# parsakzr/medvae-disentangled-multimodal

Measured on AMD Instinct MI355X. Metric: training images/sec (whole node) + ELBO parity, multimodal CVAE 64×64 bs=256, higher is better.
Workload: dtype fp32 (3xBF16 MFMA, fp32 accumulate); 1 GPU; ConditionalVAE 64x64x3 train step (fwd+loss+bwd+clip+adamw); model=ConditionalVAE, params=927333315, global_batch=256, per_gpu_batch=256, resolution=64, parallelism=dp1, rccl_world_size=1, step_launch=eager

## Files before the change

### include/medvae_hip.h

```cpp
#ifndef MEDVAE_HIP_H
#define MEDVAE_HIP_H

#include <stddef.h>

#ifdef __cplusplus
extern "C" {
#endif

#define MVAE_OK 0
#define MVAE_EINVAL (-1)
#define MVAE_EWORKSPACE (-2)

const char* mvae_last_error(void);
int mvae_abi_version(void);

int mvae_set_math_mode(int mode);
int mvae_get_math_mode(void);
int mvae_set_dropout_salt(const void* salt_dev);

#define MVAE_CONV_WSPLIT 16
#define MVAE_CONV_XSPLIT 32
#define MVAE_CONV_DYSPLIT 64
#define MVAE_CONV_BF16 128
#define MVAE_CONV_PLANAR 256
int mvae_conv2d_nhwc(const float* x, const float* w, const float* bias, const float* residual, float* y,
                     int nb, int h, int w_, int cin, int cout, int kh, int kw, int stride, int pad_t,
                     int pad_l, int ho, int wo, int mode, void* stream);
#define MVAE_CONV_DGRAD_DIRECT 512
int mvae_conv2d_direct32_nhwc(const float* x, const float* w, const float* bias, const float* residual, float* y,
                              int n, int h, int w_, int mode, void* stream);
int mvae_conv2d_ws_nhwc(const float* x, const float* w, const float* bias, const float* residual, float* y,
                        int nb, int h, int w_, int cin, int cout, int kh, int kw, int stride, int pad_t,
                        int pad_l, int ho, int wo, int mode, float* workspace, size_t workspace_bytes, void* stream);
size_t mvae_conv2d_split_workspace_bytes(int nb, int cin, int cout, int kh, int kw, int ho, int wo);
int mvae_conv2d_gnstats_nhwc(const float* x, const float* w, const float* bias, const float* residual, float* y,
                             int nb, int h, int w_, int cin, int cout, int kh, int kw, int stride, int pad_t,
                             int pad_l, int ho, int wo, int mode, double* gn_part, void* stream);

int mvae_conv2d_dgrad_gnbwd_nhwc(const float* dy, const float* wt, float* dx, int nb, int ho, int wo, int cout,
                                 int cin, int kh, int kw, int pad_t, int pad_l, int h, int w_, int w_split,
                                 const float* gn_x, const float* mean, const float* rstd, const float* gamma,
                                 const float* beta, int groups, int silu, double* part, void* stream);

int mvae_conv2d_wgrad_nhwc(const float* dy, const float* x, float* dw, float* dbias, float beta, int nb, int h, int w_,
                           int cin, int cout, int kh, int kw, int stride, int pad_t, int pad_l, int ho,
                           int wo, int mode, float* workspace, size_t workspace_bytes, void* stream);
size_t mvae_conv2d_wgrad_workspace_bytes(int nb, int cin, int cout, int kh, int kw, int ho, int wo);

int mvae_conv2d_wgrad_small_cout_nhwc(const float* dy, const float* x, float* dw, float* dbias, float beta, int nb,
                                      int h, int w_, int cin, int cout, int x_split, void* workspace,
                                      size_t workspace_bytes, void* stream);
size_t mvae_conv2d_wgrad_small_cout_workspace_bytes(int nb, int cin);
int mvae_conv2d_wgrad_direct_nhwc(const float* dy, const float* x, float* dw, float* dbias, float beta, int nb, int h,
                                  int w, int cin, int cout, int x_split, void* workspace, size_t workspace_bytes,
                                  void* stream);
size_t mvae_conv2d_wgrad_direct_workspace_bytes(int nb, int h, int w, int cin, int cout);

int mvae_conv2d_dgrad_stride2_nhwc(const float* dy, const float* wt, float* dx, int nb, int h, int w_, int cin,
                                   int cout, int kh, int kw, int pad_t, int pad_l, int ho, int wo, int w_split,
                                   float* workspace, size_t workspace_bytes, void* stream);

int mvae_conv2d_upsample_nhwc(const float* x, const float* w4, const float* bias, const float* residual, float* y,
                              int nb, int h, int w_, int cin, int cout, int w_split, void* stream);
int mvae_conv_weight_upsample_fwd(const float* w, float* w4, int cout, int cin, int split, void* stream);
int mvae_conv2d_wgrad_upsample_nhwc(const float* dy, const float* x, float* dw, float* dbias, float beta, int nb,
                                    int h, int w_, int cin, int cout, float* workspace, size_t workspace_bytes,
                                    void* stream);
size_t mvae_conv2d_wgrad_upsample_workspace_bytes(int nb, int h, int w_, int cin, int cout);

int mvae_winograd_weight_transform(const float* w, void* u, int cin, int cout, int dgrad, int tile, void* stream);
int mvae_winograd_input_transform(const float* x, void* v, int nb, int h, int w, int c, int x_split, int tile,
                                  void* stream);
int mvae_winograd_input_transform_gn(const float* x, const float* scale, const float* shift, int silu, void* v, int nb,
                                     int h, int w, int c, int tile, void* stream);
int mvae_winograd_gemm(const void* v, const void* u, float* m, long long tiles, int k_in, int n_out, int tile,
                       void* stream);
int mvae_winograd_output_transform(const float* m, const float* bias, const float* residual, float* y, double* gn_part,
                                   int nb, int h, int w, int n, int tile, void* stream);
int mvae_winograd_output_gnbwd(const float* m, float* dx, const float* x, const float* mean, const float* rstd,
                               const float* gamma, const float* beta, int groups, int silu, double* part, int nb, int h,
                               int w, int n, int tile, void* stream);
int mvae_winograd_dy_transform(const float* dy, void* d, int nb, int h, int w, int k, int dy_split, int tile,
                               void* stream);
int mvae_winograd_dy_transforms(const float* dy, void* v, void* d, int nb, int h, int w, int k, int dy_split, int tile,
                                void* stream);
int mvae_winograd_wgrad_gemm(const void* d, const void* v, float* m, long long tiles, int cout, int cin, int tile,
                             float* workspace, size_t workspace_bytes, void* stream);
int mvae_winograd_wgrad_output(const float* m, float* dw, float beta, int cout, int cin, int tile, void* stream);
int mvae_winograd_upsample_weights(const float* w, float* kc, int cin, int cout, void* stream);
int mvae_winograd_upsample_fold(const float* dkc, float* dw, float beta, int cin, int cout, void* stream);
int mvae_winograd_output_transform_upsample(const float* m, const float* bias, float* y, int nb, int h, int w, int cout,
                                            int tile, void* stream);
int mvae_winograd_dy_transforms_upsample(const float* dy, void* v, void* d, int nb, int h, int w, int cout, int tile,
                                         void* stream);

int mvae_split_bf16(const float* x, void* y, long long n, void* stream);
int mvae_pack_bf16(const float* x, void* y, long long n, void* stream);
int mvae_pack_bf16_colsum(const float* x, void* y, long long rows, int n, float* out, float beta, void* workspace,
                          size_t workspace_bytes, void* stream);
int mvae_split_planar(const float* x, void* y, long long n, void* stream);
int mvae_split_planar_colsum(const float* x, void* y, long long rows, int n, float* out, float beta, void* workspace,
                             size_t workspace_bytes, void* stream);

int mvae_conv_weight_transpose(const float* w, float* wt, int cout, int kh, int kw, int cin, int split, void* stream);
typedef struct {
  const float* w;
  float* wt;
  int cout, rs, cin, split;
  int block0, pad0;
} mvae_wt_desc;
int mvae_conv_weight_transpose_batched(const mvae_wt_desc* table, int n, int total_blocks, void* stream);
int mvae_conv_weight_upsample_dgrad(const float* w, float* wt, int cout, int cin, int split, void* stream);

int mvae_bias_grad(const float* x, long long rows, int n, long long ld, float* out, float beta,
                   void* workspace, size_t workspace_bytes, void* stream);
size_t mvae_bias_grad_workspace_bytes(long long rows, int n);

int mvae_gemm_strided_batched(int trans_a, int trans_b, int m, int n, int k, float alpha,
                              const float* A, long long lda, long long stride_a, const float* B,
                              long long ldb, long long stride_b, float beta, float* C, long long ldc,
                              long long stride_c, int batch, const float* bias, const float* residual,
                              long long ldr, long long stride_r, float* workspace,
                              size_t workspace_bytes, void* stream);
size_t mvae_gemm_workspace_bytes(int m, int n, int k, int batch);

int mvae_softmax_rows(const float* x, float* y, long long rows, int n, void* stream);
int mvae_softmax_rows_bwd(const float* y, const float* dy, float* dx, long long rows, int n, void* stream);

int mvae_attention_small_fwd(const float* q, const float* k, const float* v, float* o, float* lse, int batch, int n,
                             int c, float scale, void* stream);
int mvae_attention_small_bwd(const float* q, const float* k, const float* v, const float* dout, const float* lse,
                             float* dq, float* dk, float* dv, int batch, int n, int c, float scale, void* stream);

size_t mvae_linattn_workspace_bytes(int batch, int n, int c);
int mvae_linattn_kstats(const float* k, long long ldk, long long stride_k, float* stats, int batch, int n, int c,
                        void* workspace, size_t workspace_bytes, void* stream);
int mvae_linattn_ksoftmax(const float* k, long long ldk, long long stride_k, const float* stats, float* ksm, int batch,
                          int n, int c, void* stream);
int mvae_linattn_dk(const float* k, long long ldk, long long stride_k, const float* stats, float* dk, long long lddk,
                    long long stride_dk, int batch, int n, int c, void* workspace, size_t workspace_bytes,
                    void* stream);

int mvae_group_norm_fwd_nhwc(const float* x, const float* gamma, const float* beta, float* y, float* mean,
                             float* rstd, int nb, int hw, int c, int groups, float eps, int silu,
                             float drop_p, unsigned long long seed, int y_split, void* workspace,
                             size_t workspace_bytes, void* stream);
int mvae_group_norm_bwd_nhwc(const float* x, const float* dy, const float* gamma, const float* beta,
                             const float* mean, const float* rstd, float* dx, const float* dx_add,
                             float* dgamma, float* dbeta,
                             int nb, int hw, int c, int groups, int silu, float drop_p,
                             unsigned long long seed, void* workspace, size_t workspace_bytes,
                             void* stream);
size_t mvae_group_norm_workspace_bytes(int nb, int hw, int c);
int mvae_group_norm_bwd_pack_nhwc(const float* x, const float* dy, const float* gamma, const float* beta,
                                  const float* mean, const float* rstd, float* dx, const float* dx_add, float* dgamma,
                                  float* dbeta, int nb, int hw, int c, int groups, int silu, float drop_p,
                                  unsigned long long seed, void* workspace, size_t workspace_bytes, void* dx_packed,
                                  float* dbias, float bias_beta, void* cs_workspace, size_t cs_workspace_bytes,
                                  void* stream);
size_t mvae_group_norm_colsum_workspace_bytes(int nb, int hw, int c);
int mvae_group_norm_bwd_colsum_nhwc(const float* x, const float* dy, const float* gamma, const float* beta,
                                    const float* mean, const float* rstd, float* dx, const float* dx_add, float* dgamma,
                                    float* dbeta, int nb, int hw, int c, int groups, int silu, float drop_p,
                                    unsigned long long seed, void* workspace, size_t workspace_bytes, float* dbias,
                                    float bias_beta, void* cs_workspace, size_t cs_workspace_bytes, void* stream);
int mvae_group_norm_bwd_split_nhwc(const float* x, const float* dy, const float* gamma, const float* beta,
                                   const float* mean, const float* rstd, float* dx, const float* dx_add, float* dgamma,
                                   float* dbeta, int nb, int hw, int c, int groups, int silu, float drop_p,
                                   unsigned long long seed, void* workspace, size_t workspace_bytes, void* dx_split,
                                   float* dbias, float bias_beta, void* cs_workspace, size_t cs_workspace_bytes,
                                   void* stream);
int mvae_set_group_norm_path(int mode);
int mvae_group_norm_stats_nhwc(const float* x, const double* part, const float* gamma, const float* beta, float* mean,
                               float* rstd, float* scale, float* shift, int nb, int hw, int c, int groups, float eps,
                               void* workspace, size_t workspace_bytes, void* stream);
int mvae_group_norm_apply_nhwc(const float* x, const float* scale, const float* shift, float* y, int nb, int hw, int c,
                               int silu, int y_split, void* stream);
int mvae_group_norm_bwd_part_nhwc(const float* x, const float* dy, const double* part, const float* gamma,
                                  const float* beta, const float* mean, const float* rstd, float* dx,
                                  const float* dx_add, float* dgamma, float* dbeta, int nb, int hw, int c, int groups,
                                  int silu, void* workspace, size_t workspace_bytes, void* stream);
int mvae_group_norm_bwd_part_split_nhwc(const float* x, const float* dy, const double* part, const float* gamma,
                                        const float* beta, const float* mean, const float* rstd, float* dx,
                                        const float* dx_add, float* dgamma, float* dbeta, int nb, int hw, int c,
                                        int groups, int silu, void* workspace, size_t workspace_bytes, void* dx_split,
                                        float* dbias, float bias_beta, void* cs_workspace, size_t cs_workspace_bytes,
                                        void* stream);
int mvae_group_norm_bwd_streaming(int nb, int hw, int c, int groups, int with_dxp);
int mvae_group_norm_fwd_part_nhwc(const float* x, const double* part, const float* gamma, const float* beta, float* y,
                                  float* mean, float* rstd, int nb, int hw, int c, int groups, float eps, int silu,
                                  float drop_p, unsigned long long seed, int y_split, void* workspace,
                                  size_t workspace_bytes, void* stream);

int mvae_reparam_fwd(const float* mu, const float* logvar, long long ld, const float* eps, float* z,
                     long long npix, int zc, void* stream);
int mvae_reparam_bwd(const float* dz, const float* eps, const float* logvar, long long ld, float* dlogvar,
                     long long npix, int zc, void* stream);
int mvae_loss_reduce(int kind, const float* a, const float* b, long long ld, long long npix, int zc,
                     double scale, float* out, void* workspace, size_t workspace_bytes, void* stream);
size_t mvae_reduce_workspace_bytes(void);
int mvae_kl_bwd(const float* mu, const float* logvar, long long ld, const float* gscale, double mult,
                float* dmu, float* dlogvar, long long npix, int zc, void* stream);
int mvae_recon_bwd(int kind, const float* a, const float* b, const float* gscale, double mult, float* da,
                   long long n, void* stream);
int mvae_latent_prep_fwd(const float* h_mu, const float* h_logvar, long long ld, const float* eps, float* mu,
                         float* logvar, float* std_out, float* z, long long npix, int zc, void* stream);
int mvae_latent_prep_bwd(const float* h_mu, const float* h_logvar, long long ld, const float* eps, const float* g_mu,
                         const float* g_logvar, const float* g_std, const float* g_z, float* d_mu, float* d_logvar,
                         long long ld_out, long long npix, int zc, void* stream);
int mvae_loss_combine4_fwd(const float* v0, const float* v1, const float* v2, const float* v3, float w0, float w1,
                           float w2, float w3, int nt, float nonfinite_total, float* total, float* o0, float* o1,
                           float* o2, float* o3, float* flags, void* stream);
int mvae_loss_combine4_bwd(const float* flags, float w0, float w1, float w2, float w3, int nt, const float* g_total,
                           const float* g0, const float* g1, const float* g2, const float* g3, float* g_terms,
                           void* stream);

int mvae_multi_tensor_adam(float* params, float* grads, float* exp_avg, float* exp_avg_sq,
                           const int* chunk_tensor, const long long* chunk_start, const int* chunk_len,
                           int nchunks, const int* tensor_chunk_begin, int ntensors, const int* used,
                           int* step, float grad_scale, float max_norm, int do_clip, double lr, double beta1,
                           double beta2, float eps, double weight_decay, int decoupled, void* workspace,
                           size_t workspace_bytes, float* scalars, void* stream);
size_t mvae_multi_tensor_adam_workspace_bytes(int nchunks, int ntensors);
int mvae_multi_tensor_adam_ema(float* params, float* grads, float* exp_avg, float* exp_avg_sq,
                               const int* chunk_tensor, const long long* chunk_start, const int* chunk_len,
                               int nchunks, const int* tensor_chunk_begin, int ntensors, const int* used,
                               int* step, float grad_scale, float max_norm, int do_clip, double lr, double beta1,
                               double beta2, float eps, double weight_decay, int decoupled, void* workspace,
                               size_t workspace_bytes, float* scalars, float* ema, double ema_decay, void* stream);
int mvae_swap_buffers(float* a, float* b, size_t n, void* stream);

int mvae_lpips_scale(const float* x, float* y, long long n, int c, float a, float b, const float* shift,
                     const float* inv_scale, void* stream);
int mvae_lpips_scale_bwd(const float* dy, float* dx, long long n, int c, float a, const float* inv_scale,
                         void* stream);
int mvae_relu_fwd(const float* x, float* y, long long n, void* stream);
int mvae_relu_bwd(const float* y, const float* dy, float* dx, long long n, void* stream);
int mvae_maxpool_fwd(const float* x, float* y, unsigned char* argmax, int nb, int h, int w, int c, int k, int stride,
                     void* stream);
int mvae_maxpool_bwd(const float* dy, const unsigned char* argmax, float* dx, int nb, int h, int w, int c, int k,
                     int stride, void* stream);
int mvae_lpips_dist(const float* f0, const float* f1, const float* w, float* score, int nb, int npix, int c,
                    float beta, void* stream);
int mvae_lpips_dist_bwd(const float* f0, const float* f1, const float* w, const float* gscore, float* df0, float* df1,
                        int nb, int npix, int c, void* stream);

int mvae_ssim(const float* x, const float* y, int nb, int h, int w, int c, float data_range, float* per_image,
              void* stream);
int mvae_kl_stats(const float* mu, const float* logvar, long long ld, long long npix, int zc, float* out,
                  void* workspace, size_t workspace_bytes, void* stream);
size_t mvae_kl_stats_workspace_bytes(long long npix);
int mvae_latent_stats(const float* z, long long ld, long long stride_image, int batch, int pixels, int channels,
                      float* out, void* workspace, size_t workspace_bytes, void* stream);
size_t mvae_latent_stats_workspace_bytes(int batch, int pixels, int channels);

int mvae_decode_batch(const unsigned char* store, const long long* sample_offset, const int* sample_channels,
                      const int* sample_target_channels, const int* sample_modality, const long long* sample_label,
                      const long long* index, const float* aug, int nb, int h, int w, int cout, int n_modalities,
                      float* x, float* onehot, long long* modality_idx, long long* labels, void* workspace,
                      size_t workspace_bytes, void* stream);
size_t mvae_decode_batch_workspace_bytes(int nb, int h);

int mvae_adv_bwd(int kind, const float* a, const float* gscale, double mult, float* da, long long n, void* stream);

int mvae_batch_norm_fwd_nhwc(const float* x, const float* gamma, const float* beta, float* y, float* mean, float* rstd,
                             float* run_mean, float* run_var, long long rows, int c, float eps, float momentum,
                             int training, float slope, void* workspace, size_t workspace_bytes, void* stream);
int mvae_batch_norm_bwd_nhwc(const float* x, const float* y, const float* dy, const float* gamma, const float* mean,
                             const float* rstd, float* dx, float* dgamma, float* dbeta, long long rows, int c,
                             float slope, void* workspace, size_t workspace_bytes, void* stream);
// ... 41 lines not shown
```

### medvae_disentangled_multimodal_amd/_lib.py

```python
from __future__ import annotations

import ctypes
import os
from ctypes import c_double, c_float, c_int, c_longlong, c_size_t, c_uint64, c_void_p

_HERE = os.path.dirname(os.path.abspath(__file__))
LIB_PATH = os.environ.get("MVAE_HIP_LIB", os.path.join(_HERE, "libmvae_hip.so"))

P = c_void_p
I = c_int
L = c_longlong
F = c_float
D = c_double
Z = c_size_t

SIGNATURES = {
    "mvae_last_error": (ctypes.c_char_p, []),
    "mvae_abi_version": (I, []),
    "mvae_set_math_mode": (I, [I]),
    "mvae_get_math_mode": (I, []),
    "mvae_set_dropout_salt": (I, [P]),
    "mvae_conv2d_nhwc": (I, [P, P, P, P, P, I, I, I, I, I, I, I, I, I, I, I, I, I, P]),
    "mvae_conv2d_direct32_nhwc": (I, [P, P, P, P, P, I, I, I, I, P]),
    "mvae_conv2d_ws_nhwc": (I, [P, P, P, P, P, I, I, I, I, I, I, I, I, I, I, I, I, I, P, Z, P]),
    "mvae_conv2d_split_workspace_bytes": (Z, [I, I, I, I, I, I, I]),
    "mvae_conv2d_gnstats_nhwc": (I, [P, P, P, P, P, I, I, I, I, I, I, I, I, I, I, I, I, I, P, P]),
    "mvae_conv2d_dgrad_gnbwd_nhwc": (I, [P, P, P, I, I, I, I, I, I, I, I, I, I, I, I, P, P, P, P, P, I, I, P, P]),
    "mvae_conv2d_wgrad_nhwc": (I, [P, P, P, P, F, I, I, I, I, I, I, I, I, I, I, I, I, I, P, Z, P]),
    "mvae_winograd_weight_transform": (I, [P, P, I, I, I, I, P]),
    "mvae_winograd_input_transform": (I, [P, P, I, I, I, I, I, I, P]),
    "mvae_winograd_input_transform_gn": (I, [P, P, P, I, P, I, I, I, I, I, P]),
    "mvae_group_norm_stats_nhwc": (I, [P, P, P, P, P, P, P, P, I, I, I, I, F, P, Z, P]),
    "mvae_group_norm_apply_nhwc": (I, [P, P, P, P, I, I, I, I, I, P]),
    "mvae_winograd_gemm": (I, [P, P, P, L, I, I, I, P]),
    "mvae_winograd_output_transform": (I, [P, P, P, P, P, I, I, I, I, I, P]),
    "mvae_winograd_output_gnbwd": (I, [P, P, P, P, P, P, P, I, I, P, I, I, I, I, I, P]),
    "mvae_winograd_dy_transform": (I, [P, P, I, I, I, I, I, I, P]),
    "mvae_winograd_dy_transforms": (I, [P, P, P, I, I, I, I, I, I, P]),
    "mvae_winograd_wgrad_gemm": (I, [P, P, P, L, I, I, I, P, Z, P]),
    "mvae_winograd_wgrad_output": (I, [P, P, F, I, I, I, P]),
    "mvae_winograd_upsample_weights": (I, [P, P, I, I, P]),
    "mvae_winograd_upsample_fold": (I, [P, P, F, I, I, P]),
    "mvae_winograd_output_transform_upsample": (I, [P, P, P, I, I, I, I, I, P]),
    "mvae_winograd_dy_transforms_upsample": (I, [P, P, P, I, I, I, I, I, P]),
    "mvae_conv2d_wgrad_workspace_bytes": (Z, [I, I, I, I, I, I, I]),
    "mvae_conv2d_wgrad_small_cout_nhwc": (I, [P, P, P, P, F, I, I, I, I, I, I, P, Z, P]),
    "mvae_conv2d_wgrad_small_cout_workspace_bytes": (Z, [I, I]),
    "mvae_conv2d_wgrad_direct_nhwc": (I, [P, P, P, P, F, I, I, I, I, I, I, P, Z, P]),
    "mvae_conv2d_wgrad_direct_workspace_bytes": (Z, [I, I, I, I, I]),
    "mvae_conv_weight_transpose": (I, [P, P, I, I, I, I, I, P]),
    "mvae_conv_weight_transpose_batched": (I, [P, I, I, P]),
    "mvae_conv_weight_upsample_dgrad": (I, [P, P, I, I, I, P]),
    "mvae_conv2d_dgrad_stride2_nhwc": (I, [P, P, P, I, I, I, I, I, I, I, I, I, I, I, I, P, Z, P]),
    "mvae_split_bf16": (I, [P, P, L, P]),
    "mvae_pack_bf16": (I, [P, P, L, P]),
    "mvae_pack_bf16_colsum": (I, [P, P, L, I, P, F, P, Z, P]),
    "mvae_split_planar": (I, [P, P, L, P]),
    "mvae_split_planar_colsum": (I, [P, P, L, I, P, F, P, Z, P]),
    "mvae_conv2d_upsample_nhwc": (I, [P, P, P, P, P, I, I, I, I, I, I, P]),
    "mvae_conv_weight_upsample_fwd": (I, [P, P, I, I, I, P]),
    "mvae_conv2d_wgrad_upsample_nhwc": (I, [P, P, P, P, F, I, I, I, I, I, P, Z, P]),
    "mvae_conv2d_wgrad_upsample_workspace_bytes": (Z, [I, I, I, I, I]),
    "mvae_bias_grad": (I, [P, L, I, L, P, F, P, Z, P]),
    "mvae_bias_grad_workspace_bytes": (Z, [L, I]),
    "mvae_gemm_strided_batched": (I, [I, I, I, I, I, F, P, L, L, P, L, L, F, P, L, L, I, P, P, L, L, P, Z, P]),
    "mvae_gemm_workspace_bytes": (Z, [I, I, I, I]),
    "mvae_softmax_rows": (I, [P, P, L, I, P]),
    "mvae_softmax_rows_bwd": (I, [P, P, P, L, I, P]),
    "mvae_attention_small_fwd": (I, [P, P, P, P, P, I, I, I, F, P]),
    "mvae_attention_small_bwd": (I, [P, P, P, P, P, P, P, P, I, I, I, F, P]),
    "mvae_linattn_workspace_bytes": (Z, [I, I, I]),
    "mvae_linattn_kstats": (I, [P, L, L, P, I, I, I, P, Z, P]),
    "mvae_linattn_ksoftmax": (I, [P, L, L, P, P, I, I, I, P]),
    "mvae_linattn_dk": (I, [P, L, L, P, P, L, L, I, I, I, P, Z, P]),
    "mvae_group_norm_fwd_nhwc": (I, [P, P, P, P, P, P, I, I, I, I, F, I, F, c_uint64, I, P, Z, P]),
    "mvae_group_norm_fwd_part_nhwc": (I, [P, P, P, P, P, P, P, I, I, I, I, F, I, F, c_uint64, I, P, Z, P]),
    "mvae_group_norm_bwd_nhwc": (I, [P, P, P, P, P, P, P, P, P, P, I, I, I, I, I, F, c_uint64, P, Z, P]),
    "mvae_group_norm_bwd_part_nhwc": (I, [P, P, P, P, P, P, P, P, P, P, P, I, I, I, I, I, P, Z, P]),
    "mvae_group_norm_bwd_part_split_nhwc": (I, [P, P, P, P, P, P, P, P, P, P, P, I, I, I, I, I, P, Z, P, P, F, P, Z,
                                               P]),
    "mvae_group_norm_bwd_streaming": (I, [I, I, I, I, I]),
    "mvae_group_norm_workspace_bytes": (Z, [I, I, I]),
    "mvae_group_norm_bwd_pack_nhwc": (I, [P, P, P, P, P, P, P, P, P, P, I, I, I, I, I, F, c_uint64, P, Z, P, P, F, P, Z,
                                          P]),
    "mvae_group_norm_bwd_split_nhwc": (I, [P, P, P, P, P, P, P, P, P, P, I, I, I, I, I, F, c_uint64, P, Z, P, P, F, P, Z,
                                          P]),
    "mvae_group_norm_bwd_colsum_nhwc": (I, [P, P, P, P, P, P, P, P, P, P, I, I, I, I, I, F, c_uint64, P, Z, P, F, P, Z,
                                           P]),
    "mvae_group_norm_colsum_workspace_bytes": (Z, [I, I, I]),
    "mvae_set_group_norm_path": (I, [I]),
    "mvae_reparam_fwd": (I, [P, P, L, P, P, L, I, P]),
    "mvae_reparam_bwd": (I, [P, P, P, L, P, L, I, P]),
    "mvae_loss_reduce": (I, [I, P, P, L, L, I, D, P, P, Z, P]),
    "mvae_reduce_workspace_bytes": (Z, []),
    "mvae_kl_bwd": (I, [P, P, L, P, D, P, P, L, I, P]),
    "mvae_latent_prep_fwd": (I, [P, P, L, P, P, P, P, P, L, I, P]),
    "mvae_latent_prep_bwd": (I, [P, P, L, P, P, P, P, P, P, P, L, L, I, P]),
    "mvae_loss_combine4_fwd": (I, [P, P, P, P, F, F, F, F, I, F, P, P, P, P, P, P, P]),
    "mvae_loss_combine4_bwd": (I, [P, F, F, F, F, I, P, P, P, P, P, P, P]),
    "mvae_recon_bwd": (I, [I, P, P, P, D, P, L, P]),
    "mvae_multi_tensor_adam": (I, [P, P, P, P, P, P, P, I, P, I, P, P, F, F, I, D, D, D, F, D, I, P, Z, P, P]),
    "mvae_multi_tensor_adam_workspace_bytes": (Z, [I, I]),
    "mvae_multi_tensor_adam_ema": (I, [P, P, P, P, P, P, P, I, P, I, P, P, F, F, I, D, D, D, F, D, I, P, Z, P, P, D,
                                       P]),
    "mvae_swap_buffers": (I, [P, P, Z, P]),
    "mvae_lpips_scale": (I, [P, P, L, I, F, F, P, P, P]),
    "mvae_lpips_scale_bwd": (I, [P, P, L, I, F, P, P]),
    "mvae_relu_fwd": (I, [P, P, L, P]),
    "mvae_relu_bwd": (I, [P, P, P, L, P]),
    "mvae_maxpool_fwd": (I, [P, P, P, I, I, I, I, I, I, P]),
    "mvae_maxpool_bwd": (I, [P, P, P, I, I, I, I, I, I, P]),
    "mvae_lpips_dist": (I, [P, P, P, P, I, I, I, F, P]),
    "mvae_lpips_dist_bwd": (I, [P, P, P, P, P, P, I, I, I, P]),
    "mvae_ssim": (I, [P, P, I, I, I, I, F, P, P]),
    "mvae_kl_stats": (I, [P, P, L, L, I, P, P, Z, P]),
    "mvae_kl_stats_workspace_bytes": (Z, [L]),
    "mvae_latent_stats": (I, [P, L, L, I, I, I, P, P, Z, P]),
    "mvae_latent_stats_workspace_bytes": (Z, [I, I, I]),
    "mvae_decode_batch": (I, [P, P, P, P, P, P, P, P, I, I, I, I, I, P, P, P, P, P, Z, P]),
    "mvae_decode_batch_workspace_bytes": (Z, [I, I]),
    "mvae_adv_bwd": (I, [I, P, P, D, P, L, P]),
# ... 91 lines not shown
```

### medvae_disentangled_multimodal_amd/csrc/norm.hip

```cpp
#include "common.h"
#include <algorithm>
#include <stdlib.h>

namespace mvae {

#ifndef GN_UNROLL
#define GN_UNROLL 4
#endif

__device__ __forceinline__ float4 gn_ld4(const float* p) {
#ifndef GN_TEMPORAL
  const f32x4 v = __builtin_nontemporal_load((const f32x4*)p);
  return float4{v[0], v[1], v[2], v[3]};
#else
  return *(const float4*)p;
#endif
}

__device__ __forceinline__ float hash_uniform(unsigned long long seed, unsigned long long idx) {
  unsigned long long z = seed + 0x9E3779B97F4A7C15ull * (idx + 1);
  z = (z ^ (z >> 30)) * 0xBF58476D1CE4E5B9ull;
  z = (z ^ (z >> 27)) * 0x94D049BB133111EBull;
  z ^= z >> 31;
  return (float)(unsigned)(z >> 40) * (1.0f / 16777216.0f);
// ... 193 lines not shown
    mean[i] = (float)mu;
    rstd[i] = rs;
  }
  for (int c = g * cpg + lane; c < (g + 1) * cpg; c += 64) {
    const float sc = rs * a.gamma[c];
    scale[b * a.C + c] = sc;
    shift[b * a.C + c] = a.beta[c] - (float)mu * sc;
  }
}

__global__ void __launch_bounds__(256) gn_apply_kernel(GnArgs a, const float* __restrict__ scale,
                                                       const float* __restrict__ shift, float* __restrict__ y) {
  const int b = blockIdx.y;
  const long long sbase = (long long)b * a.hw * a.C;
  for (int cg0 = 0; cg0 < (a.C >> 2); cg0 += 256) {
    GnMap mp(a, cg0);
    if (mp.act) {
      const float4 sc = *(const float4*)(scale + (long long)b * a.C + mp.c4 * 4);
      const float4 sh = *(const float4*)(shift + (long long)b * a.C + mp.c4 * 4);
      const float* xp = a.x + sbase + mp.c4 * 4;
      float* yp = y + sbase + mp.c4 * 4;
      for (int row = mp.row_lo + mp.rph; row < mp.row_hi; row += GN_UNROLL * mp.rpar) {
        float4 xv[GN_UNROLL];
#pragma unroll
        for (int u = 0; u < GN_UNROLL; ++u) {
          const int r = row + u * mp.rpar;
          xv[u] = r < mp.row_hi ? gn_ld4(xp + (long long)r * a.C) : float4{0.f, 0.f, 0.f, 0.f};
        }
#pragma unroll
        for (int u = 0; u < GN_UNROLL; ++u) {
          const int r = row + u * mp.rpar;
          if (r >= mp.row_hi) continue;
          float o[4] = {xv[u].x * sc.x + sh.x, xv[u].y * sc.y + sh.y, xv[u].z * sc.z + sh.z, xv[u].w * sc.w + sh.w};
          const long long off = sbase + (long long)r * a.C + mp.c4 * 4;
#pragma unroll
          for (int k = 0; k < 4; ++k) {
            if (a.silu) o[k] = o[k] * sigmoid_f(o[k]);
            if (a.drop_p > 0.f) {
              const float uu = hash_uniform(drop_seed(a), (unsigned long long)(off + k));
              o[k] = (uu >= a.drop_p) ? o[k] / (1.f - a.drop_p) : 0.f;
            }
          }
          const float4 ov{o[0], o[1], o[2], o[3]};
          if (a.y_split >= 2) {
            const unsigned h01 = pk_bf16x2(ov.x, ov.y), h23 = pk_bf16x2(ov.z, ov.w);
            *(uint2*)((__bf16*)y + off) = uint2{h01, h23};
            if (a.y_split == 3)
              *(uint2*)((__bf16*)y + (long long)a.nb * a.hw * a.C + off) =
                  uint2{pk_bf16x2(ov.x - __uint_as_float(h01 << 16), ov.y - __uint_as_float(h01 & 0xFFFF0000u)),
                        pk_bf16x2(ov.z - __uint_as_float(h23 << 16), ov.w - __uint_as_float(h23 & 0xFFFF0000u))};
          } else if (a.y_split)
            *(uint4*)(yp + (long long)r * a.C) = split4_bf16(ov);
          else
            *(float4*)(yp + (long long)r * a.C) = ov;
        }
      }
    }
    if ((a.C >> 2) < 256) break;
  }
}

__global__ void __launch_bounds__(256) gn_bwd_finalize_kernel(GnArgs a, float* k1, float* k2, float* k3) {
  const int i = blockIdx.x * 4 + (threadIdx.x >> 6), lane = threadIdx.x & 63;
  if (i >= a.nb * a.G) return;
  const int b = i / a.G, g = i - b * a.G;
  const int cpg = a.C / a.G;
  double A1 = 0, A2 = 0;
  for (int j = lane; j < a.chunks * cpg; j += 64) {
    const int ch = j / cpg, c = g * cpg + (j - ch * cpg);
    const double* w = a.ws + (((long long)b * a.chunks + ch) * a.C + c) * 2;
    A1 += (double)a.gamma[c] * w[0];
    A2 += (double)a.gamma[c] * w[1];
  }
  A1 = wave_sum_d(A1);
  A2 = wave_sum_d(A2);
  const float rsf = a.rstd[i];
  for (int c = g * cpg + lane; c < (g + 1) * cpg; c += 64) k1[b * a.C + c] = rsf * a.gamma[c];
  if (lane == 0) {
    const double n = (double)a.hw * cpg;
    const double rs = rsf, mu = a.mean[i];
    k2[i] = (float)(-rs * rs * A2 / n);
    k3[i] = (float)(-rs * A1 / n + mu * rs * rs * A2 / n);
  }
}

constexpr int GN_PG_SLICES = 64;
__global__ void __launch_bounds__(256) gn_param_grad_kernel(GnArgs a, double* __restrict__ part) {
  __shared__ double sh[2][256];
  const int cl = threadIdx.x & 63, rg = threadIdx.x >> 6;
  const int c = blockIdx.x * 64 + cl, sl = blockIdx.y;
  const int n = a.nb * a.chunks;
  const int lo = (int)((long long)n * sl / GN_PG_SLICES), hi = (int)((long long)n * (sl + 1) / GN_PG_SLICES);
  double s0 = 0, s1 = 0;
  if (c < a.C) {
    for (int i = lo + rg; i < hi; i += 4) {
      const double* w = a.ws + ((long long)i * a.C + c) * 2;
      s0 += w[0];
      s1 += w[1];
    }
  }
  sh[0][threadIdx.x] = s0;
  sh[1][threadIdx.x] = s1;
  __syncthreads();
  if (rg == 0 && c < a.C) {
    double* o = part + ((long long)sl * a.C + c) * 2;
    o[0] = sh[0][cl] + sh[0][cl + 64] + sh[0][cl + 128] + sh[0][cl + 192];
    o[1] = sh[1][cl] + sh[1][cl + 64] + sh[1][cl + 128] + sh[1][cl + 192];
  }
}

__global__ void __launch_bounds__(256) gn_param_final_kernel(int C, const double* __restrict__ part,
                                                              float* dgamma, float* dbeta) {
  const int c = blockIdx.x * 256 + threadIdx.x;
  if (c >= C) return;
  double s0 = 0, s1 = 0;
  for (int sl = 0; sl < GN_PG_SLICES; ++sl) {
    s0 += part[((long long)sl * C + c) * 2];
    s1 += part[((long long)sl * C + c) * 2 + 1];
  }
  if (dgamma) dgamma[c] += (float)s1;
  if (dbeta) dbeta[c] += (float)s0;
}

__global__ void __launch_bounds__(256) gn_dx_kernel(GnArgs a, const float* __restrict__ k1,
                                                    const float* __restrict__ k2, const float* __restrict__ k3,
                                                    float* __restrict__ dx) {
  const int b = blockIdx.y;
  const int cpg = a.C / a.G;
  const long long sbase = (long long)b * a.hw * a.C;
  __shared__ double csr[256][4];
  for (int cg0 = 0; cg0 < (a.C >> 2); cg0 += 256) {
    GnMap mp(a, cg0);
    double cs[4] = {0.0, 0.0, 0.0, 0.0};
    if (mp.act) {
      float m[4], rs[4], gm[4], bt[4], q1[4], q2[4], q3[4];
#pragma unroll
      for (int e = 0; e < 4; ++e) {
        const int c = mp.c4 * 4 + e, bg = b * a.G + c / cpg;
        m[e] = a.mean[bg];
        rs[e] = a.rstd[bg];
        gm[e] = a.gamma[c];
        bt[e] = a.beta[c];
        q1[e] = k1[(long long)b * a.C + c];
        q2[e] = k2[bg];
        q3[e] = k3[bg];
      }
      const float* xp = a.x + sbase + mp.c4 * 4;
      const float* dp = a.dy + sbase + mp.c4 * 4;
      float* op = dx + sbase + mp.c4 * 4;
      const float* ap = a.dx_add ? a.dx_add + sbase + mp.c4 * 4 : nullptr;
      for (int row = mp.row_lo + mp.rph; row < mp.row_hi; row += GN_UNROLL * mp.rpar) {
        float4 xv[GN_UNROLL], dv[GN_UNROLL], av[GN_UNROLL];
#pragma unroll
        for (int u = 0; u < GN_UNROLL; ++u) {
          const int r = row + u * mp.rpar;
          const bool ok = r < mp.row_hi;
          xv[u] = ok ? gn_ld4(xp + (long long)r * a.C) : float4{0.f, 0.f, 0.f, 0.f};
          dv[u] = ok ? gn_ld4(dp + (long long)r * a.C) : float4{0.f, 0.f, 0.f, 0.f};
          av[u] = (ap != nullptr && ok) ? gn_ld4(ap + (long long)r * a.C) : float4{0.f, 0.f, 0.f, 0.f};
        }
#pragma unroll
        for (int u = 0; u < GN_UNROLL; ++u) {
          const int r = row + u * mp.rpar;
          if (r >= mp.row_hi) continue;
          const float xs[4] = {xv[u].x, xv[u].y, xv[u].z, xv[u].w};
          const float ds[4] = {dv[u].x, dv[u].y, dv[u].z, dv[u].w};
// ... 855 lines not shown
    set_error("group_norm_bwd: bad geometry");
    return MVAE_EINVAL;
  }
  if (dx == nullptr && dxp == nullptr) {
    set_error("group_norm_bwd: dx may be null only when the split / packed copy is written");
    return MVAE_EINVAL;
  }
  if (workspace_bytes < mvae_group_norm_workspace_bytes(nb, hw, c)) {
    set_error("group_norm_bwd: workspace too small");
    return MVAE_EWORKSPACE;
  }
  hipStream_t st = (hipStream_t)stream;
  GnArgs a{};
  a.x = x; a.dy = dy; a.mean = mean; a.rstd = rstd; a.gamma = gamma; a.beta = beta; a.dx_add = dx_add;
  a.nb = nb; a.hw = hw; a.C = c; a.G = groups; a.silu = silu; a.drop_p = drop_p; a.seed = seed; a.salt = dropout_salt();
  a.chunks = gn_chunks(nb, hw);
  a.rows_per_chunk = (hw + a.chunks - 1) / a.chunks;
  a.ws = (double*)workspace;
  a.dxp = (uint2*)dxp;
  a.dxp_split = dxp_split;
  a.csp = dbias ? (double*)cs_ws : nullptr;
  int it = 0;
  static const int bwd_max_it = [] {
    const char* e = getenv("MVAE_GN_RES_BWD_IT");
    return e ? std::min(13, atoi(e)) : 13;
  }();
  int sc = gn_resident_slab(nb, hw, c, groups, &it, bwd_max_it);
  if (sc > 0 && sc < 32 && (long long)nb * hw * c * 4 > (64LL << 20)) sc = 0;
  if (sc) {
    double* pws = (double*)workspace;
    const int units = nb * (c / sc);
    const void* k = it == 4 ? (const void*)gn_bwd_resident_kernel<4>
                  : it == 8 ? (const void*)gn_bwd_resident_kernel<8> : (const void*)gn_bwd_resident_kernel<13>;
    const dim3 grid(gn_res_grid(k, units));
    if (it == 4) hipLaunchKernelGGL(gn_bwd_resident_kernel<4>, grid, dim3(GN_RES_NT), 0, st, a, sc, units, pws, dx);
    else if (it == 8) hipLaunchKernelGGL(gn_bwd_resident_kernel<8>, grid, dim3(GN_RES_NT), 0, st, a, sc, units, pws, dx);
    else hipLaunchKernelGGL(gn_bwd_resident_kernel<13>, grid, dim3(GN_RES_NT), 0, st, a, sc, units, pws, dx);
    if (dgamma || dbeta)
      hipLaunchKernelGGL(gn_param_reduce_kernel, dim3(c), dim3(256), 0, st, (const double*)pws, nb, c, dgamma, dbeta);
    if (dbias)
      hipLaunchKernelGGL(gn_colsum_final_kernel, dim3(cdiv(c, 16)), dim3(256), 0, st, (const double*)a.csp, nb, c,
                         dbias, bias_beta);
    return launch_status();
  }
  if (const int sc2 = (dxp || dbias) ? 0 : gn_unit2_slab(hw, c, groups)) {
    double* pws = (double*)workspace;
    const int units = nb * (c / sc2);
    int dev = 0, cus = 0;
    (void)hipGetDevice(&dev);
    (void)hipDeviceGetAttribute(&cus, hipDeviceAttributeMultiprocessorCount, dev);
    static const int per_cu = [] {
      const char* e = getenv("MVAE_GN_UNIT_PER_CU");
      return e ? std::max(1, atoi(e)) : 1;
    }();
    const dim3 grid(std::max(1, std::min(units, std::max(1, cus) * per_cu)));
    hipLaunchKernelGGL(gn_bwd_unit2_kernel<4>, grid, dim3(GN_RES_NT), 0, st, a, sc2, units, pws, dx);
    if (dgamma || dbeta)
      hipLaunchKernelGGL(gn_param_reduce_kernel, dim3(c), dim3(256), 0, st, (const double*)pws, nb, c, dgamma, dbeta);
    return launch_status();
  }
  float* k1 = (float*)((char*)workspace + (size_t)nb * a.chunks * c * 2 * sizeof(double));
  float* k2 = k1 + (size_t)nb * c;
  float* k3 = k2 + (size_t)nb * c;
  hipLaunchKernelGGL(gn_partial_kernel<1>, dim3(a.chunks, nb), dim3(256), 0, st, a);
  hipLaunchKernelGGL(gn_bwd_finalize_kernel, dim3(cdiv((long long)nb * groups, 4)), dim3(256), 0, st, a, k1,
                     k2, k3);
  if (dgamma || dbeta) {
    double* part = (double*)(((uintptr_t)(k3 + (size_t)nb * c) + 255) & ~(uintptr_t)255);
    hipLaunchKernelGGL(gn_param_grad_kernel, dim3(cdiv(c, 64), GN_PG_SLICES), dim3(256), 0, st, a, part);
    hipLaunchKernelGGL(gn_param_final_kernel, dim3(cdiv(c, 256)), dim3(256), 0, st, c, (const double*)part, dgamma,
                       dbeta);
  }
  hipLaunchKernelGGL(gn_dx_kernel, dim3(a.chunks, nb), dim3(256), 0, st, a, k1, k2, k3, dx);
  if (dbias)
    hipLaunchKernelGGL(gn_colsum_final_kernel, dim3(cdiv(c, 16)), dim3(256), 0, st, (const double*)a.csp,
                       nb * a.chunks, c, dbias, bias_beta);
  return launch_status();
}

static int gn_bwd_part(const float* x, const float* dy, const double* part, const float* gamma, const float* beta,
                       const float* mean, const float* rstd, float* dx, const float* dx_add, float* dgamma,
                       float* dbeta, int nb, int hw, int c, int groups, int silu, void* workspace,
                       size_t workspace_bytes, void* dx_split, float* dbias, float bias_beta, void* cs_ws,
                       void* stream);

int mvae_group_norm_bwd_part_nhwc(const float* x, const float* dy, const double* part, const float* gamma,
                                  const float* beta, const float* mean, const float* rstd, float* dx,
                                  const float* dx_add, float* dgamma, float* dbeta, int nb, int hw, int c, int groups,
                                  int silu, void* workspace, size_t workspace_bytes, void* stream) {
  return gn_bwd_part(x, dy, part, gamma, beta, mean, rstd, dx, dx_add, dgamma, dbeta, nb, hw, c, groups, silu,
                     workspace, workspace_bytes, nullptr, nullptr, 0.f, nullptr, stream);
}

int mvae_group_norm_bwd_part_split_nhwc(const float* x, const float* dy, const double* part, const float* gamma,
                                        const float* beta, const float* mean, const float* rstd, float* dx,
                                        const float* dx_add, float* dgamma, float* dbeta, int nb, int hw, int c,
                                        int groups, int silu, void* workspace, size_t workspace_bytes, void* dx_split,
                                        float* dbias, float bias_beta, void* cs_workspace, size_t cs_workspace_bytes,
                                        void* stream) {
  if ((dx_split == nullptr && dbias == nullptr) || ((uintptr_t)dx_split & 15) || ((uintptr_t)dx & 15) ||
      ((uintptr_t)x & 15) || ((uintptr_t)dy & 15) || (dx_add && ((uintptr_t)dx_add & 15)) ||
      (dbias && cs_workspace == nullptr)) {
    set_error("group_norm_bwd_part_split: 16-B aligned x / dy / dx / split output (or a bias gradient), a column-sum "
              "workspace");
    return MVAE_EINVAL;
  }
  if (dbias && cs_workspace_bytes < mvae_group_norm_colsum_workspace_bytes(nb, hw, c)) {
    set_error("group_norm_bwd_part_split: column-sum workspace too small");
    return MVAE_EWORKSPACE;
  }
  return gn_bwd_part(x, dy, part, gamma, beta, mean, rstd, dx, dx_add, dgamma, dbeta, nb, hw, c, groups, silu,
                     workspace, workspace_bytes, dx_split, dbias, bias_beta, cs_workspace, stream);
}

int mvae_group_norm_bwd_streaming(int nb, int hw, int c, int groups, int with_dxp) {
  if (nb <= 0 || hw <= 0 || c <= 0 || (c & 3) || groups <= 0 || c % groups) return 0;
  static const int bwd_max_it = [] {
    const char* e = getenv("MVAE_GN_RES_BWD_IT");
    return e ? std::min(13, atoi(e)) : 13;
  }();
  int it = 0;
  int sc = gn_resident_slab(nb, hw, c, groups, &it, bwd_max_it);
  if (sc > 0 && sc < 32 && (long long)nb * hw * c * 4 > (64LL << 20)) sc = 0;
  if (sc) return 0;
  return (with_dxp || !gn_unit2_slab(hw, c, groups)) ? 1 : 0;
}

static int gn_bwd_part(const float* x, const float* dy, const double* part, const float* gamma, const float* beta,
                       const float* mean, const float* rstd, float* dx, const float* dx_add, float* dgamma,
                       float* dbeta, int nb, int hw, int c, int groups, int silu, void* workspace,
                       size_t workspace_bytes, void* dx_split, float* dbias, float bias_beta, void* cs_ws,
                       void* stream) {
  if (nb <= 0 || hw <= 0 || c <= 0 || (c & 3) || groups <= 0 || c % groups || hw % 32 || part == nullptr) {
    set_error("group_norm_bwd_part: needs hw %% 32 == 0 and C %% 4 == 0");
    return MVAE_EINVAL;
  }
  if (dx == nullptr && dx_split == nullptr) {
    set_error("group_norm_bwd_part: dx may be null only when the split copy is written");
    return MVAE_EINVAL;
  }
  if (workspace_bytes < mvae_group_norm_workspace_bytes(nb, hw, c)) {
    set_error("group_norm_bwd_part: workspace too small");
    return MVAE_EWORKSPACE;
  }
  hipStream_t st = (hipStream_t)stream;
  GnArgs a{};
  a.x = x; a.dy = dy; a.mean = mean; a.rstd = rstd; a.gamma = gamma; a.beta = beta; a.dx_add = dx_add;
  a.nb = nb; a.hw = hw; a.C = c; a.G = groups; a.silu = silu; a.drop_p = 0.f; a.seed = 0;
  a.chunks = gn_chunks(nb, hw);
  a.rows_per_chunk = (hw + a.chunks - 1) / a.chunks;
  a.dxp = (uint2*)dx_split;
  a.dxp_split = 1;
  a.csp = dbias ? (double*)cs_ws : nullptr;
  float* k1 = (float*)((char*)workspace + (size_t)nb * a.chunks * c * 2 * sizeof(double));
  float* k2 = k1 + (size_t)nb * c;
  float* k3 = k2 + (size_t)nb * c;
  GnArgs ap = a;
  ap.ws = const_cast<double*>(part);
  ap.chunks = hw / 32;
  ap.rows_per_chunk = 32;
  hipLaunchKernelGGL(gn_bwd_finalize_kernel, dim3(cdiv((long long)nb * groups, 4)), dim3(256), 0, st, ap, k1,
                     k2, k3);
  if (dgamma || dbeta) {
    double* pg = (double*)(((uintptr_t)(k3 + (size_t)nb * c) + 255) & ~(uintptr_t)255);
    hipLaunchKernelGGL(gn_param_grad_kernel, dim3(cdiv(c, 64), GN_PG_SLICES), dim3(256), 0, st, ap, pg);
    hipLaunchKernelGGL(gn_param_final_kernel, dim3(cdiv(c, 256)), dim3(256), 0, st, c, (const double*)pg, dgamma,
                       dbeta);
  }
  hipLaunchKernelGGL(gn_dx_kernel, dim3(a.chunks, nb), dim3(256), 0, st, a, k1, k2, k3, dx);
  if (dbias)
    hipLaunchKernelGGL(gn_colsum_final_kernel, dim3(cdiv(c, 16)), dim3(256), 0, st, (const double*)a.csp,
                       nb * a.chunks, c, dbias, bias_beta);
  return launch_status();
}

}

namespace mvae {
__global__ void __launch_bounds__(256) softmax_rows_kernel(const float* __restrict__ x, float* __restrict__ y,
                                                           long long rows, int n) {
  const long long row = blockIdx.x * 4LL + (threadIdx.x >> 6);
  const int lane = threadIdx.x & 63;
  if (row >= rows) return;
  const float* xr = x + row * n;
  float* yr = y + row * n;
  float m = -INFINITY;
  for (int j = lane; j < n; j += 64) m = fmaxf(m, xr[j]);
  m = wave_max_f(m);
  float s = 0.f;
  for (int j = lane; j < n; j += 64) s += __expf(xr[j] - m);
  s = wave_sum_f(s);
  const float inv = 1.f / s;
  for (int j = lane; j < n; j += 64) yr[j] = __expf(xr[j] - m) * inv;
}

__global__ void __launch_bounds__(256) softmax_rows_bwd_kernel(const float* __restrict__ y,
                                                               const float* __restrict__ dy,
                                                               float* __restrict__ dx, long long rows, int n) {
  const long long row = blockIdx.x * 4LL + (threadIdx.x >> 6);
  const int lane = threadIdx.x & 63;
  if (row >= rows) return;
  const float* yr = y + row * n;
  const float* dr = dy + row * n;
  float s = 0.f;
  for (int j = lane; j < n; j += 64) s += yr[j] * dr[j];
  s = wave_sum_f(s);
  for (int j = lane; j < n; j += 64) dx[row * n + j] = yr[j] * (dr[j] - s);
}
}

extern "C" {
int mvae_softmax_rows(const float* x, float* y, long long rows, int n, void* stream) {
  if (rows <= 0 || n <= 0) { set_error("softmax: bad sizes"); return MVAE_EINVAL; }
  hipLaunchKernelGGL(softmax_rows_kernel, dim3((unsigned)((rows + 3) / 4)), dim3(256), 0, (hipStream_t)stream, x,
                     y, rows, n);
  return launch_status();
}
int mvae_softmax_rows_bwd(const float* y, const float* dy, float* dx, long long rows, int n, void* stream) {
  if (rows <= 0 || n <= 0) { set_error("softmax_bwd: bad sizes"); return MVAE_EINVAL; }
  hipLaunchKernelGGL(softmax_rows_bwd_kernel, dim3((unsigned)((rows + 3) / 4)), dim3(256), 0, (hipStream_t)stream,
                     y, dy, dx, rows, n);
  return launch_status();
}
}
```

### medvae_disentangled_multimodal_amd/csrc/winograd.hip

```cpp
#include "gemm_core.h"

namespace mvae {

__device__ __forceinline__ float4 f4add(float4 a, float4 b) { return float4{a.x + b.x, a.y + b.y, a.z + b.z, a.w + b.w}; }

template <int MT>
__host__ __device__ constexpr float wino_bt(int i, int j) {
  if constexpr (MT == 2) {
    constexpr float m[4][4] = {{1, 0, -1, 0}, {0, 1, 1, 0}, {0, -1, 1, 0}, {0, 1, 0, -1}};
    return m[i][j];
  } else {
    constexpr float m[6][6] = {{4, 0, -5, 0, 1, 0},  {0, -4, -4, 1, 1, 0}, {0, 4, -4, -1, 1, 0},
                               {0, -2, -1, 2, 1, 0}, {0, 2, -1, -2, 1, 0}, {0, 4, 0, -5, 0, 1}};
    return m[i][j];
  }
}
template <int MT>
__host__ __device__ constexpr float wino_g(int i, int j) {
  if constexpr (MT == 2) {
    constexpr float m[4][3] = {{1, 0, 0}, {0.5f, 0.5f, 0.5f}, {0.5f, -0.5f, 0.5f}, {0, 0, 1}};
    return m[i][j];
  } else {
    constexpr float m[6][3] = {{0.25f, 0, 0},
                               {-1.f / 6, -1.f / 6, -1.f / 6},
// ... 346 lines not shown
  if constexpr (ST) {
    __shared__ double2 sm[TW][MT][CG];
#pragma unroll
    for (int a = 0; a < MT; ++a) sm[wt][a][cl] = double2{s0[a], s1[a]};
    __syncthreads();
    const int q = threadIdx.x / CG, cb = chunk * CG + cl;
    if (q < NBK && cb < N4) {
      double2 s = double2{0.0, 0.0};
      for (int wr = q * RPB; wr < (q + 1) * RPB; ++wr)
#pragma unroll
        for (int tq = 0; tq < CT; ++tq) {
          const double2 v = sm[(wr / MT) * CT + tq][wr % MT][cl];
          s.x += v.x;
          s.y += v.y;
        }
      const long long blk = (((long long)b * p.H + ti0 * MT + q * RPB) * p.W + seg * WSEG) >> 5;
      *(double2*)(p.gn_part + (blk * N4 + cb) * 2) = s;
    }
  }
  if constexpr (GNB) {
    __shared__ float2 sg[TW][MT][CG][4];
#pragma unroll
    for (int a = 0; a < MT; ++a)
#pragma unroll
      for (int u = 0; u < 4; ++u) sg[wt][a][cl][u] = float2{g0[a][u], g1[a][u]};
    __syncthreads();
    for (int i = threadIdx.x; i < NBK * CG * 4; i += 256) {
      const int u = i & 3, cc = (i >> 2) % CG, q = i / (4 * CG), cb = chunk * CG + cc;
      if (cb >= N4) continue;
      double d0 = 0.0, d1 = 0.0;
      for (int wr = q * RPB; wr < (q + 1) * RPB; ++wr)
#pragma unroll
        for (int tq = 0; tq < CT; ++tq) {
          const float2 v = sg[(wr / MT) * CT + tq][wr % MT][cc][u];
          d0 += (double)v.x;
          d1 += (double)v.y;
        }
      const long long blk = (((long long)b * p.H + ti0 * MT + q * RPB) * p.W + seg * WSEG) >> 5;
      *(double2*)(p.gnb_part + (blk * N + cb * 4 + u) * 2) = double2{d0, d1};
    }
  }
}

template <int MT>
__global__ void __launch_bounds__(256) wino_out_any_kernel(WinoOut p) {
  constexpr int AL = MT + 2;
  const int N = p.N, N4 = N >> 2, th = (p.H + MT - 1) / MT, tw = (p.W + MT - 1) / MT;
  const long long T = (long long)p.nb * th * tw;
  const unsigned mplane = (unsigned)(T * N4 * 16);
  const __amdgpu_buffer_rsrc_t mr = make_rsrc(p.m, mplane * (unsigned)(AL * AL));
  const long long idx = (long long)blockIdx.x * blockDim.x + threadIdx.x;
  if (idx >= T * N4) return;
  const long long t = idx / N4;
  const int c4 = (int)(idx - t * N4);
  const int tj = (int)(t % tw), ti = (int)((t / tw) % th), b = (int)(t / ((long long)tw * th));
  const float4 bv = p.bias ? *(const float4*)(p.bias + c4 * 4) : float4{0.f, 0.f, 0.f, 0.f};
  float4 mv[AL][AL];
#pragma unroll
  for (int i = 0; i < AL; ++i)
#pragma unroll
    for (int j = 0; j < AL; ++j) mv[i][j] = bload4(mr, (unsigned)(t * N4 + c4) * 16u + (unsigned)(i * AL + j) * mplane);
  constexpr auto at = [](int i, int k) { return wino_at<MT>(i, k); };
  float4 r[MT][AL];
#pragma unroll
  for (int j = 0; j < AL; ++j) wlin<MT, AL>(&r[0][j], AL, &mv[0][j], AL, at);
#pragma unroll
  for (int a = 0; a < MT; ++a) {
    float4 o[MT];
    wlin<MT, AL>(o, 1, &r[a][0], 1, at);
    const int row = ti * MT + a;
#pragma unroll
    for (int e = 0; e < MT; ++e) {
      const int col = tj * MT + e;
      if (row < p.H && col < p.W) {
        const long long off = (((long long)b * p.H + row) * p.W + col) * N + c4 * 4;
        float4 val = f4add(o[e], bv);
        if (p.res) val = f4add(val, *(const float4*)(p.res + off));
        *(float4*)(p.y + off) = val;
      }
    }
  }
}

template <bool UPS>
struct DySrc {
  unsigned pix0, chan, rowb;
  int H, W;
  __device__ DySrc(int b, int k4, int H_, int W_, int K) : H(H_), W(W_) {
    if constexpr (UPS) {
      const int cq4 = K >> 4, pq = k4 / cq4, c4 = k4 - pq * cq4;
      pix0 = (unsigned)((b * 2 * H + (pq >> 1)) * 2 * W + (pq & 1));
      chan = (unsigned)c4 * 16u;
      rowb = (unsigned)(K >> 2) * 4u;
    } else {
      pix0 = (unsigned)(b * H * W);
      chan = (unsigned)k4 * 16u;
      rowb = (unsigned)K * 4u;
    }
  }
  __device__ unsigned off(int h, int w) const {
    if constexpr (UPS) return (pix0 + (unsigned)(2 * h * 2 * W + 2 * w)) * rowb + chan;
    else return (pix0 + (unsigned)(h * W + w)) * rowb + chan;
  }
};

template <int MT, bool XS, int SF = 0, bool UPS = false>
__global__ void __launch_bounds__(256) wino_dy_kernel(const float* __restrict__ dy, uint4* __restrict__ d, int nb, int H,
                                                      int W, int K) {
  constexpr int AL = MT + 2;
  const int K4 = K >> 2, th = (H + MT - 1) / MT, tw = (W + MT - 1) / MT;
  const long long T = (long long)nb * th * tw;
  const long long idx = (long long)blockIdx.x * blockDim.x + threadIdx.x;
  if (idx >= T * K4) return;
  const long long t = idx / K4;
  const int k4 = (int)(idx - t * K4);
  const int tj = (int)(t % tw), ti = (int)((t / tw) % th), b = (int)(t / ((long long)tw * th));
  const __amdgpu_buffer_rsrc_t dr = make_rsrc(dy, (unsigned)((long long)nb * H * W * K * 4));
  const DySrc<UPS> src(b, k4, H, W, K);
  const unsigned plane = (unsigned)(T * K4) * wgb<SF>(), base = (unsigned)(t * K4 + k4) * wgb<SF>();
  const __amdgpu_buffer_rsrc_t vr = make_rsrc(d, plane * (unsigned)(AL * AL));
  float4 v[MT][MT];
#pragma unroll
  for (int a = 0; a < MT; ++a)
#pragma unroll
    for (int e = 0; e < MT; ++e) {
      const int h = MT * ti + a, w = MT * tj + e;
      const float4 r = bload4(dr, (h < H && w < W) ? src.off(h, w) : OOB);
      v[a][e] = XS ? split4_to_f32(r) : r;
    }
  constexpr auto ac = [](int i, int k) { return wino_at<MT>(k, i); };
  float4 c[AL][MT], o[AL][AL];
#pragma unroll
  for (int e = 0; e < MT; ++e) wlin<AL, MT>(&c[0][e], MT, &v[0][e], MT, ac);
#pragma unroll
  for (int i = 0; i < AL; ++i) wlin<AL, MT>(&o[i][0], 1, &c[i][0], 1, ac);
#pragma unroll
  for (int i = 0; i < AL; ++i)
#pragma unroll
    for (int j = 0; j < AL; ++j) wstore_f<SF>(vr, base + (unsigned)(i * AL + j) * plane, o[i][j]);
}

template <int MT, bool XS, int SF = 0, bool UPS = false>
__global__ void __launch_bounds__(256) wino_dy2_kernel(const float* __restrict__ dy, uint4* __restrict__ v,
                                                       uint4* __restrict__ d, int nb, int H, int W, int K) {
  constexpr int AL = MT + 2;
  const int K4 = K >> 2, th = (H + MT - 1) / MT, tw = (W + MT - 1) / MT;
  const long long T = (long long)nb * th * tw;
  const long long idx = (long long)blockIdx.x * blockDim.x + threadIdx.x;
  if (idx >= T * K4) return;
  const long long t = idx / K4;
  const int k4 = (int)(idx - t * K4);
  const int tj = (int)(t % tw), ti = (int)((t / tw) % th), b = (int)(t / ((long long)tw * th));
  const __amdgpu_buffer_rsrc_t xr = make_rsrc(dy, (unsigned)((long long)nb * H * W * K * 4));
  const DySrc<UPS> src(b, k4, H, W, K);
  const unsigned plane = (unsigned)(T * K4) * wgb<SF>(), base = (unsigned)(t * K4 + k4) * wgb<SF>();
  const __amdgpu_buffer_rsrc_t vr = make_rsrc(v, plane * (unsigned)(AL * AL));
  const __amdgpu_buffer_rsrc_t dr = make_rsrc(d, plane * (unsigned)(AL * AL));
  float4 p[AL][AL];
#pragma unroll
  for (int i = 0; i < AL; ++i)
#pragma unroll
    for (int j = 0; j < AL; ++j) {
      const int h = MT * ti - 1 + i, w = MT * tj - 1 + j;
      const bool ok = (unsigned)h < (unsigned)H && (unsigned)w < (unsigned)W;
      const float4 r = bload4(xr, ok ? src.off(h, w) : OOB);
      p[i][j] = XS ? split4_to_f32(r) : r;
    }
#pragma unroll
  for (int i = 0; i < AL; ++i) {
    float4 ci[MT], o[AL];
#pragma unroll
    for (int e = 0; e < MT; ++e) {
      bool first = true;
      ci[e] = float4{0.f, 0.f, 0.f, 0.f};
#pragma unroll
      for (int u = 0; u < MT; ++u) wmadd(ci[e], first, wino_at<MT>(u, i), p[1 + u][1 + e]);
    }
#pragma unroll
    for (int j = 0; j < AL; ++j) {
      bool first = true;
      o[j] = float4{0.f, 0.f, 0.f, 0.f};
#pragma unroll
      for (int e = 0; e < MT; ++e) wmadd(o[j], first, wino_at<MT>(e, j), ci[e]);
    }
#pragma unroll
    for (int j = 0; j < AL; ++j) wstore_f<SF>(dr, base + (unsigned)(i * AL + j) * plane, o[j]);
  }
  constexpr auto bt = [](int i, int k) { return wino_bt<MT>(i, k); };
#pragma unroll
  for (int j = 0; j < AL; ++j) wlin<AL, AL>(&p[0][j], AL, &p[0][j], AL, bt);
#pragma unroll
  for (int i = 0; i < AL; ++i) wlin<AL, AL>(&p[i][0], 1, &p[i][0], 1, bt);
#pragma unroll
  for (int i = 0; i < AL; ++i)
#pragma unroll
    for (int j = 0; j < AL; ++j) wstore_f<SF>(vr, base + (unsigned)(i * AL + j) * plane, p[i][j]);
}

__host__ __device__ constexpr int ups_tap(int p, int r) { return p == 0 ? (r == 0 ? 0 : 1) : (r == 2 ? 2 : 1); }

__global__ void __launch_bounds__(256) wino_ups_weights_kernel(const float* __restrict__ w, float* __restrict__ kc,
                                                               int cout, int cin) {
  const int C4 = cin >> 2;
  const long long idx = (long long)blockIdx.x * blockDim.x + threadIdx.x;
  if (idx >= 4LL * cout * C4) return;
  const int c4 = (int)(idx % C4);
  const long long kq = idx / C4;
  const int k = (int)(kq % cout), pq = (int)(kq / cout), p = pq >> 1, q = pq & 1;
  float4 o[3][3];
#pragma unroll
  for (int a = 0; a < 3; ++a)
#pragma unroll
    for (int bb = 0; bb < 3; ++bb) o[a][bb] = float4{0.f, 0.f, 0.f, 0.f};
#pragma unroll
  for (int r = 0; r < 3; ++r)
#pragma unroll
    for (int s2 = 0; s2 < 3; ++s2) {
      const float4 v = *(const float4*)(w + (((long long)k * 3 + r) * 3 + s2) * cin + c4 * 4);
      o[ups_tap(p, r)][ups_tap(q, s2)] = f4add(o[ups_tap(p, r)][ups_tap(q, s2)], v);
    }
#pragma unroll
  for (int a = 0; a < 3; ++a)
#pragma unroll
    for (int bb = 0; bb < 3; ++bb) *(float4*)(kc + ((kq * 3 + a) * 3 + bb) * cin + c4 * 4) = o[a][bb];
}

__global__ void __launch_bounds__(256) wino_ups_fold_kernel(const float* __restrict__ dkc, float* __restrict__ dw,
                                                            float beta, int cout, int cin) {
  const int C4 = cin >> 2;
  const long long idx = (long long)blockIdx.x * blockDim.x + threadIdx.x;
  if (idx >= (long long)cout * C4) return;
  const int k = (int)(idx / C4), c4 = (int)(idx - (long long)k * C4);
#pragma unroll
  for (int r = 0; r < 3; ++r)
#pragma unroll
    for (int s2 = 0; s2 < 3; ++s2) {
      float4 acc = float4{0.f, 0.f, 0.f, 0.f};
#pragma unroll
      for (int pq = 0; pq < 4; ++pq) {
        const long long row = (long long)pq * cout + k;
        acc = f4add(acc, *(const float4*)(dkc + ((row * 3 + ups_tap(pq >> 1, r)) * 3 + ups_tap(pq & 1, s2)) * cin +
                                          c4 * 4));
      }
      float4* q = (float4*)(dw + (((long long)k * 3 + r) * 3 + s2) * cin + c4 * 4);
      if (beta != 0.f) {
        const float4 old = *q;
        acc = float4{fmaf(beta, old.x, acc.x), fmaf(beta, old.y, acc.y), fmaf(beta, old.z, acc.z),
                     fmaf(beta, old.w, acc.w)};
      }
      *q = acc;
    }
}

template <int MT>
__global__ void __launch_bounds__(256) wino_out_ups_kernel(WinoOut p) {
  constexpr int AL = MT + 2;
  const int N = p.N, N4 = N >> 2, K4 = N, th = (p.H + MT - 1) / MT, tw = (p.W + MT - 1) / MT;
  const long long T = (long long)p.nb * th * tw;
  const unsigned mplane = (unsigned)(T * K4 * 16);
  const __amdgpu_buffer_rsrc_t mr = make_rsrc(p.m, mplane * (unsigned)(AL * AL));
  const long long idx = (long long)blockIdx.x * blockDim.x + threadIdx.x;
  if (idx >= T * K4) return;
  const long long t = idx / K4;
  const int k4 = (int)(idx - t * K4), pq = k4 / N4, c4 = k4 - pq * N4;
  const int tj = (int)(t % tw), ti = (int)((t / tw) % th), b = (int)(t / ((long long)tw * th));
  const float4 bv = p.bias ? *(const float4*)(p.bias + c4 * 4) : float4{0.f, 0.f, 0.f, 0.f};
  const __amdgpu_buffer_rsrc_t yr = make_rsrc(p.y, (unsigned)((long long)p.nb * 4 * p.H * p.W * N * 4));
  float4 mv[AL][AL];
#pragma unroll
  for (int i = 0; i < AL; ++i)
#pragma unroll
    for (int j = 0; j < AL; ++j) mv[i][j] = bload4(mr, (unsigned)(t * K4 + k4) * 16u + (unsigned)(i * AL + j) * mplane);
  constexpr auto at = [](int i, int k) { return wino_at<MT>(i, k); };
  float4 r[MT][AL];
#pragma unroll
  for (int j = 0; j < AL; ++j) wlin<MT, AL>(&r[0][j], AL, &mv[0][j], AL, at);
#pragma unroll
  for (int a = 0; a < MT; ++a) {
    float4 o[MT];
// ... 43 lines not shown
      *q = val;
    }
}

static long long wino_tiles(int nb, int h, int w, int mt) {
  return (long long)nb * ((h + mt - 1) / mt) * ((w + mt - 1) / mt);
}

static bool wino_geom_ok(int mt, int nb, int h, int w, int cin, int cout) {
  return (mt == 2 || mt == 4) && nb > 0 && h > 0 && w > 0 && cin > 0 && cout > 0 && cin % 4 == 0 && cout % 4 == 0 &&
         (long long)nb * h * w * std::max(cin, cout) * 4 <= MAX_DESC_BYTES &&
         (long long)(mt + 2) * (mt + 2) * wino_tiles(nb, h, w, mt) * std::max(cin, cout) * 4 <= MAX_DESC_BYTES;
}

static bool wino_blocks_ok(int h, int w) { return h % 4 == 0 && (w == 8 || w == 16 || (w >= 32 && w % 32 == 0)); }

static int egrid256(long long n) { return (int)std::min<long long>((n + 255) / 256, 1LL << 30); }

static int wino_sf() { return math_mode() == MATH_FP32 ? 1 : math_mode() == MATH_BF16 ? 2 : 0; }
static bool wino_split_in_ok(int split) {
  if (!split || wino_sf() != 1) return true;
  set_error("winograd: pre-split (3xBF16) inputs are not used in the exact fp32 arithmetic");
  return false;
}

#define WINO_GO(FN, MT, ...)                        \
  do {                                              \
    if (sf == 1) FN<MT, 1>(__VA_ARGS__);            \
    else if (sf == 2) FN<MT, 2>(__VA_ARGS__);       \
    else FN<MT, 0>(__VA_ARGS__);                    \
  } while (0)

template <int MT, int SF>
static void wt_go(const float* w, void* u, int cin, int cout, int dgrad, hipStream_t st) {
  if (dgrad) {
    if constexpr (MT == 4) {
      if ((long long)cin * cout >= (1LL << 20)) {
        hipLaunchKernelGGL((wino_wt_dgrad_kernel<4, true, SF>), dim3(cdiv(cin, WDG_N), cdiv(cout / 4, wdg_kq<4, true>())),
                           dim3(WDG_N * wdg_kq<4, true>()), 0, st, w, (uint4*)u, cout, cin);
        return;
      }
    }
    hipLaunchKernelGGL((wino_wt_dgrad_kernel<MT, false, SF>), dim3(cdiv(cin, WDG_N), cdiv(cout / 4, wdg_kq<MT, false>())),
                       dim3(WDG_N * wdg_kq<MT, false>()), 0, st, w, (uint4*)u, cout, cin);
  } else {
    hipLaunchKernelGGL((wino_wt_fwd_kernel<MT, SF>), dim3(egrid256((long long)cout * (cin / 4))), dim3(256), 0, st, w,
                       (uint4*)u, cout, cin);
  }
}

template <int MT, int SF>
static void in_go(const float* x, void* v, int nb, int h, int w, int c, int xs, int gn, WinoGn p, hipStream_t st) {
  const dim3 g(egrid256(wino_tiles(nb, h, w, MT) * (c / 4)));
  if constexpr (SF != 1) {
    if (xs) {
      hipLaunchKernelGGL((wino_in_kernel<MT, true, 0, SF>), g, dim3(256), 0, st, x, (uint4*)v, nb, h, w, c, p);
      return;
    }
  }
  if (gn == 2) hipLaunchKernelGGL((wino_in_kernel<MT, false, 2, SF>), g, dim3(256), 0, st, x, (uint4*)v, nb, h, w, c, p);
  else if (gn == 1) hipLaunchKernelGGL((wino_in_kernel<MT, false, 1, SF>), g, dim3(256), 0, st, x, (uint4*)v, nb, h, w, c, p);
  else hipLaunchKernelGGL((wino_in_kernel<MT, false, 0, SF>), g, dim3(256), 0, st, x, (uint4*)v, nb, h, w, c, p);
}

template <int MT, int SF>
static void dy_go(const float* dy, void* v, void* d, int nb, int h, int w, int k, int xs, bool both, hipStream_t st,
                  bool ups = false) {
  const dim3 g(egrid256(wino_tiles(nb, h, w, MT) * (k / 4)));
  uint4 *vv = (uint4*)v, *dd = (uint4*)d;
  if (ups) {
    if (both) hipLaunchKernelGGL((wino_dy2_kernel<MT, false, SF, true>), g, dim3(256), 0, st, dy, vv, dd, nb, h, w, k);
    else hipLaunchKernelGGL((wino_dy_kernel<MT, false, SF, true>), g, dim3(256), 0, st, dy, dd, nb, h, w, k);
    return;
  }
  if constexpr (SF != 1) {
    if (xs) {
      if (both) hipLaunchKernelGGL((wino_dy2_kernel<MT, true, SF>), g, dim3(256), 0, st, dy, vv, dd, nb, h, w, k);
      else hipLaunchKernelGGL((wino_dy_kernel<MT, true, SF>), g, dim3(256), 0, st, dy, dd, nb, h, w, k);
      return;
    }
  }
  if (both) hipLaunchKernelGGL((wino_dy2_kernel<MT, false, SF>), g, dim3(256), 0, st, dy, vv, dd, nb, h, w, k);
  else hipLaunchKernelGGL((wino_dy_kernel<MT, false, SF>), g, dim3(256), 0, st, dy, dd, nb, h, w, k);
}

template <int MT, int WSEG>
static void wino_out_go(WinoOut& p, bool gnb, hipStream_t st) {
  const dim3 g((unsigned)wino_out_blocks<MT, WSEG>(p));
  if (gnb) hipLaunchKernelGGL((wino_out_kernel<MT, WSEG, true, false>), g, dim3(256), 0, st, p);
  else if (p.gn_part) hipLaunchKernelGGL((wino_out_kernel<MT, WSEG, false, true>), g, dim3(256), 0, st, p);
  else hipLaunchKernelGGL((wino_out_kernel<MT, WSEG, false, false>), g, dim3(256), 0, st, p);
}

static int wino_out_launch(WinoOut& p, int tile, bool gnb, void* stream) {
  hipStream_t st = (hipStream_t)stream;
  if (!wino_blocks_ok(p.H, p.W)) {
    const dim3 g(egrid256(wino_tiles(p.nb, p.H, p.W, tile) * (p.N / 4)));
    if (tile == 2) hipLaunchKernelGGL(wino_out_any_kernel<2>, g, dim3(256), 0, st, p);
    else hipLaunchKernelGGL(wino_out_any_kernel<4>, g, dim3(256), 0, st, p);
    return launch_status();
  }
  const int wseg = std::min(p.W, 32);
  if (tile == 2) {
    if (wseg == 8) wino_out_go<2, 8>(p, gnb, st);
    else if (wseg == 16) wino_out_go<2, 16>(p, gnb, st);
    else wino_out_go<2, 32>(p, gnb, st);
  } else {
    if (wseg == 8) wino_out_go<4, 8>(p, gnb, st);
    else if (wseg == 16) wino_out_go<4, 16>(p, gnb, st);
    else wino_out_go<4, 32>(p, gnb, st);
  }
  return launch_status();
}

template <int CFG, int AK, int BKIND>
static bool persist_cfg(GemmArgs& a, hipStream_t st) {
  constexpr int BM = TILE_CFGS[CFG].bm, BN = TILE_CFGS[CFG].bn, WGM = TILE_CFGS[CFG].wgm, WGN = TILE_CFGS[CFG].wgn;
  a.tiles_m = cdiv(a.M, BM);
  a.tiles_n = cdiv(a.N, BN);
  const long long total = (long long)a.tiles_m * a.tiles_n * a.batch, slots = 256LL * resident_of(CFG);
  if (total <= slots || total > (1LL << 30)) return false;
  if (a.xcd_groups <= 0) a.xcd_groups = xcd_groups_env();
  const dim3 grid((unsigned)slots), block(64 * WGM * WGN);
  if (math_mode() == MATH_FP32) {
    if constexpr (CFG == T256x256) return false;
    else hipLaunchKernelGGL((gemm3x_persist_kernel<BM, BN, WGM, WGN, AK, 4, BKIND, 4, 0>), grid, block, 0, st, a);
  } else {
    hipLaunchKernelGGL((gemm3x_persist_kernel<BM, BN, WGM, WGN, AK, 4, BKIND, 4, 3>), grid, block, 0, st, a);
  }
  return true;
}
template <int AK, int BKIND>
static bool launch_persist(GemmArgs& a, hipStream_t st, int cfg) {
  static_assert(AK == A_ROWK_SPLIT && BKIND == B_ROWK_SPLIT, "persistent GEMM: pre-split ROW x ROW operands");
  if (getenv("MVAE_NO_PERSISTENT_GEMM") != nullptr || math_mode() == MATH_BF16 || a.splits != 1 || a.bias || a.res ||
      a.beta != 0.f || a.out_remap || a.gn_part || a.gnb_part || a.bias_ws || (a.N & 3) || (a.ldc & 3) || (a.sC & 3) ||
      !al16(a.C) || vec_epi_disabled())
    return false;
  if (cfg == T256x256) return persist_cfg<T256x256, AK, BKIND>(a, st);
  if (cfg == T256x128) return persist_cfg<T256x128, AK, BKIND>(a, st);
  return false;
}

}

using namespace mvae;

extern "C" {

int mvae_winograd_weight_transform(const float* w, void* u, int cin, int cout, int dgrad, int tile, void* stream) {
  if (!w || !u || cin <= 0 || cout <= 0 || cin % 4 || cout % 4 || !al16(w) || !al16(u) || (tile != 2 && tile != 4)) {
    set_error("winograd_weight_transform: cin, cout multiples of 4, 16-B aligned w / u, tile 2 or 4");
    return MVAE_EINVAL;
  }
  hipStream_t st = (hipStream_t)stream;
  const int sf = wino_sf();
  if (tile == 2) WINO_GO(wt_go, 2, w, u, cin, cout, dgrad, st);
  else WINO_GO(wt_go, 4, w, u, cin, cout, dgrad, st);
  return launch_status();
}

int mvae_winograd_input_transform(const float* x, void* v, int nb, int h, int w, int c, int x_split, int tile,
                                  void* stream) {
  if (!x || !v || !wino_geom_ok(tile, nb, h, w, c, c) || !al16(x) || !al16(v)) {
    set_error("winograd_input_transform: tile 2 or 4, c %% 4 == 0, 16-B aligned");
    return MVAE_EINVAL;
// ... 52 lines not shown
  const int cfg = choose_tile(a, true, false);
  static const bool no_tail = getenv("MVAE_NO_TAIL_SPLIT") != nullptr;
  int b_main = a.batch;
  if (!no_tail && cfg >= T256x256 && cfg <= T64x64) {
    GemmArgs one = a;
    one.batch = 1;
    const long long tp = tiles_of(cfg, one), slots = 256LL * resident_of(cfg), tot = tp * a.batch;
    const long long full = tot / slots, rem = tot - full * slots;
    if (full >= 1 && rem > 0 && rem * 2 <= slots) b_main = (int)std::max<long long>(1, full * slots / tp);
  }
  if (b_main >= a.batch) {
    go(a, cfg);
    return launch_status();
  }
  GemmArgs t = a;
  a.batch = b_main;
  go(a, cfg);
  t.batch -= b_main;
  t.A = (const float*)((const char*)t.A + (long long)b_main * t.sA * eb);
  t.B = (const float*)((const char*)t.B + (long long)b_main * t.sB * eb);
  t.C += (long long)b_main * t.sC;
  go(t, choose_tile(t, true, false));
  return launch_status();
}

int mvae_winograd_output_transform(const float* m, const float* bias, const float* residual, float* y, double* gn_part,
                                   int nb, int h, int w, int n, int tile, void* stream) {
  if (!m || !y || !wino_geom_ok(tile, nb, h, w, n, n) || !al16(m) || !al16(y) || (bias && !al16(bias)) ||
      (residual && !al16(residual)) || (gn_part && !wino_blocks_ok(h, w))) {
    set_error("winograd_output_transform: tile 2 or 4, n %% 4 == 0, 16-B aligned; statistics need h %% 4 == 0 and w in "
              "{8, 16} or a multiple of 32");
    return MVAE_EINVAL;
  }
  WinoOut p{};
  p.m = m; p.bias = bias; p.res = residual; p.y = y; p.gn_part = gn_part;
  p.groups = 1; p.nb = nb; p.H = h; p.W = w; p.N = n;
  return wino_out_launch(p, tile, false, stream);
}

int mvae_winograd_output_gnbwd(const float* m, float* dx, const float* x, const float* mean, const float* rstd,
                               const float* gamma, const float* beta, int groups, int silu, double* part, int nb, int h,
                               int w, int n, int tile, void* stream) {
  if (!m || !dx || !x || !mean || !rstd || !gamma || !beta || !part || groups <= 0 || n % groups ||
      (n / groups) % 4 || !wino_geom_ok(tile, nb, h, w, n, n) || !wino_blocks_ok(h, w) || !al16(m) || !al16(dx) ||
      !al16(x)) {
    set_error("winograd_output_gnbwd: tile 2 or 4, h %% 4 == 0, w in {8, 16} or a multiple of 32, channels per "
              "group %% 4 == 0, 16-B aligned");
    return MVAE_EINVAL;
  }
  WinoOut p{};
  p.m = m; p.y = dx; p.gnb_part = part; p.gx = x; p.mean = mean; p.rstd = rstd; p.gamma = gamma; p.beta = beta;
  p.groups = groups; p.silu = silu; p.nb = nb; p.H = h; p.W = w; p.N = n;
  return wino_out_launch(p, tile, true, stream);
}

int mvae_winograd_dy_transform(const float* dy, void* d, int nb, int h, int w, int k, int dy_split, int tile,
                               void* stream) {
  if (!dy || !d || !wino_geom_ok(tile, nb, h, w, k, k) || !al16(dy) || !al16(d)) {
    set_error("winograd_dy_transform: tile 2 or 4, k %% 4 == 0, 16-B aligned");
    return MVAE_EINVAL;
  }
  if (!wino_split_in_ok(dy_split)) return MVAE_EINVAL;
  hipStream_t st = (hipStream_t)stream;
  const int sf = wino_sf();
  if (tile == 2) WINO_GO(dy_go, 2, dy, nullptr, d, nb, h, w, k, dy_split, false, st);
  else WINO_GO(dy_go, 4, dy, nullptr, d, nb, h, w, k, dy_split, false, st);
  return launch_status();
}

int mvae_winograd_dy_transforms(const float* dy, void* v, void* d, int nb, int h, int w, int k, int dy_split, int tile,
                                void* stream) {
  if (!dy || !v || !d || !wino_geom_ok(tile, nb, h, w, k, k) || !al16(dy) || !al16(v) || !al16(d)) {
    set_error("winograd_dy_transforms: tile 2 or 4, k %% 4 == 0, 16-B aligned");
    return MVAE_EINVAL;
  }
  if (!wino_split_in_ok(dy_split)) return MVAE_EINVAL;
  hipStream_t st = (hipStream_t)stream;
  const int sf = wino_sf();
  if (tile == 2) WINO_GO(dy_go, 2, dy, v, d, nb, h, w, k, dy_split, true, st);
  else WINO_GO(dy_go, 4, dy, v, d, nb, h, w, k, dy_split, true, st);
  return launch_status();
}

int mvae_winograd_wgrad_gemm(const void* d, const void* v, float* m, long long tiles, int cout, int cin, int tile,
                             float* workspace, size_t workspace_bytes, void* stream) {
  if (!d || !v || !m || tiles <= 0 || cout <= 0 || cin <= 0 || cout % 4 || cin % 4 || !al16(d) || !al16(v) || !al16(m) ||
      tiles * std::max(cout, cin) * 4 > MAX_DESC_BYTES || tiles > (1LL << 30) || (tile != 2 && tile != 4)) {
    set_error("winograd_wgrad_gemm: cout, cin multiples of 4, 16-B aligned, one position < 4 GiB, tile 2 or 4");
    return MVAE_EINVAL;
  }
  const bool pk = wino_sf() == 2;
  if (pk && (cout % 8 || cin % 8)) {
    set_error("winograd_wgrad_gemm: the bf16 (packed) operands need cout, cin %% 8 == 0");
    return MVAE_EINVAL;
  }
  const unsigned eb = pk ? 2u : 4u;
  GemmArgs a{};
  a.M = cout; a.N = cin; a.K = (int)tiles; a.batch = (tile + 2) * (tile + 2);
  a.A = (const float*)d; a.lda = cout; a.sA = tiles * cout;
  a.B = (const float*)v; a.ldb = cin; a.sB = tiles * cin;
  a.C = m; a.ldc = cin; a.sC = (long long)cout * cin;
  a.alpha = 1.f; a.beta = 0.f;
  a.a_bytes = (unsigned)(tiles * cout * eb); a.b_bytes = (unsigned)(tiles * cin * eb);
  a.c_bytes = (unsigned)((long long)cout * cin * 4);
  const int cfg = choose_tile(a, true, workspace != nullptr);
  plan_splits(a, cfg, workspace, workspace_bytes);
  if (pk) wgrad_dma(B_COLN, a, (hipStream_t)stream, cfg, 4);
  else launch_big<A_COLM_SPLIT, 4, B_COLN_SPLIT, 4>(a, (hipStream_t)stream, cfg);
  return gemm_finish(a, (hipStream_t)stream);
}

int mvae_winograd_upsample_weights(const float* w, float* kc, int cin, int cout, void* stream) {
  if (!w || !kc || cin <= 0 || cout <= 0 || cin % 4 || !al16(w) || !al16(kc)) {
    set_error("winograd_upsample_weights: cin %% 4 == 0, 16-B aligned");
    return MVAE_EINVAL;
  }
  hipLaunchKernelGGL(wino_ups_weights_kernel, dim3(egrid256(4LL * cout * (cin / 4))), dim3(256), 0, (hipStream_t)stream,
                     w, kc, cout, cin);
  return launch_status();
}

int mvae_winograd_upsample_fold(const float* dkc, float* dw, float beta, int cin, int cout, void* stream) {
  if (!dkc || !dw || cin <= 0 || cout <= 0 || cin % 4 || !al16(dkc) || !al16(dw)) {
    set_error("winograd_upsample_fold: cin %% 4 == 0, 16-B aligned");
    return MVAE_EINVAL;
  }
  hipLaunchKernelGGL(wino_ups_fold_kernel, dim3(egrid256((long long)cout * (cin / 4))), dim3(256), 0,
                     (hipStream_t)stream, dkc, dw, beta, cout, cin);
  return launch_status();
}

int mvae_winograd_output_transform_upsample(const float* m, const float* bias, float* y, int nb, int h, int w, int cout,
                                            int tile, void* stream) {
  if (!m || !y || cout % 4 || !wino_geom_ok(tile, nb, h, w, 4 * cout, 4 * cout) || !al16(m) || !al16(y) ||
      (bias && !al16(bias)) || (long long)nb * 4 * h * w * cout * 4 > MAX_DESC_BYTES) {
    set_error("winograd_output_transform_upsample: tile 2 or 4, cout %% 4 == 0, 16-B aligned, operands < 4 GiB");
    return MVAE_EINVAL;
  }
  WinoOut p{};
  p.m = m; p.bias = bias; p.y = y;
  p.groups = 1; p.nb = nb; p.H = h; p.W = w; p.N = cout;
  const dim3 g(egrid256(wino_tiles(nb, h, w, tile) * cout));
  if (tile == 2) hipLaunchKernelGGL(wino_out_ups_kernel<2>, g, dim3(256), 0, (hipStream_t)stream, p);
  else hipLaunchKernelGGL(wino_out_ups_kernel<4>, g, dim3(256), 0, (hipStream_t)stream, p);
  return launch_status();
}

int mvae_winograd_dy_transforms_upsample(const float* dy, void* v, void* d, int nb, int h, int w, int cout, int tile,
                                         void* stream) {
  if (!dy || !d || cout % 4 || !wino_geom_ok(tile, nb, h, w, 4 * cout, 4 * cout) || !al16(dy) || !al16(d) ||
      (v && !al16(v))) {
    set_error("winograd_dy_transforms_upsample: tile 2 or 4, cout %% 4 == 0, 16-B aligned, operands < 4 GiB");
    return MVAE_EINVAL;
  }
  hipStream_t st = (hipStream_t)stream;
  const int sf = wino_sf(), k = 4 * cout;
  if (tile == 2) WINO_GO(dy_go, 2, dy, v, d, nb, h, w, k, 0, v != nullptr, st, true);
  else WINO_GO(dy_go, 4, dy, v, d, nb, h, w, k, 0, v != nullptr, st, true);
  return launch_status();
}

int mvae_winograd_wgrad_output(const float* m, float* dw, float beta, int cout, int cin, int tile, void* stream) {
  if (!m || !dw || cout <= 0 || cin <= 0 || cin % 4 || !al16(m) || !al16(dw) || (tile != 2 && tile != 4)) {
    set_error("winograd_wgrad_output: cin %% 4 == 0, 16-B aligned, tile 2 or 4");
    return MVAE_EINVAL;
  }
// ... 10 lines not shown
```

### medvae_disentangled_multimodal_amd/ops.py

```python
from __future__ import annotations

import ctypes
import math
import os
import weakref
from dataclasses import dataclass
from typing import NamedTuple, Optional, Tuple

import torch

from . import _lib

CL = torch.channels_last


def _stream(t: torch.Tensor) -> int:
    return torch.cuda.current_stream(t.device).cuda_stream


def _ptr(t: Optional[torch.Tensor]):
    return None if t is None else t.data_ptr()


def _check(t: torch.Tensor, name: str = "tensor"):
# ... 173 lines not shown
    return ref * (m + 2) ** 2 / (9.0 * m * m)


WINOGRAD_MAX_W = int(os.environ.get("MVAE_WINOGRAD_MAX_W", "64"))


WINOGRAD_MIN_MACS = float(os.environ.get("MVAE_WINOGRAD_MIN_MACS", "1e10"))


def _wino_ok(g, n: int, h: int, wd: int, cin: int, cout: int) -> bool:
    mode = _MATH[0]
    if mode == 0:
        on, maxw = _dma_fmt() == 0, WINOGRAD_MAX_W
    elif mode == 2:
        on, maxw = WINOGRAD_EXACT, WINOGRAD_MAX_W
    else:
        on, maxw = WINOGRAD_BF16, min(WINOGRAD_MAX_W, WINOGRAD_BF16_MAX_W)
    return (WINOGRAD and on and g.kh == 3 and g.kw == 3 and g.stride == 1 and
            not g.upsample and (g.pad_t, g.pad_l, g.pad_b, g.pad_r) == (1, 1, 1, 1) and wd <= maxw and
            cin % (8 if mode == 1 else 4) == 0 and cout % (8 if mode == 1 else 4) == 0 and
            min(cin, cout) >= (WINOGRAD_MIN_C_WIDE if wd >= 32 else WINOGRAD_MIN_C) and
            9.0 * n * h * wd * cin * cout >= WINOGRAD_MIN_MACS and
            len(_wino_chunks(n, h, wd, max(cin, cout))) <= WINOGRAD_MAX_CHUNKS)


_MAX_DESC_BYTES = 0xFFFFFF00

WINOGRAD_UPSAMPLE = os.environ.get("MVAE_NO_WINOGRAD_UPSAMPLE") is None
WINOGRAD_UPSAMPLE_BF16 = os.environ.get("MVAE_WINOGRAD_UPSAMPLE_BF16") is not None


def _wino_ups_ok(g, n: int, h: int, wd: int, cin: int, cout: int) -> bool:
    return (WINOGRAD_UPSAMPLE and (_MATH[0] != 1 or WINOGRAD_UPSAMPLE_BF16) and _subpixel_upsample(g) and
            h % _wtile() == 0 and wd % _wtile() == 0 and cout % 8 == 0 and _wino_ok(G3, n, h, wd, cin, 4 * cout) and
            min(cin, cout) >= (WINOGRAD_MIN_C_WIDE if wd >= 32 else WINOGRAD_MIN_C) and
            4 * n * h * wd * cout * 4 <= _MAX_DESC_BYTES)


WINOGRAD_MAX_CHUNKS = 4


def _wino_chunks(n: int, h: int, wd: int, cmax: int):
    per_img = (_wtile() + 2) ** 2 * _wino_tiles(1, h, wd) * cmax * 4
    per = max(1, _MAX_DESC_BYTES // per_img) if per_img <= _MAX_DESC_BYTES else 0
    if per == 0:
        return [None] * (WINOGRAD_MAX_CHUNKS + 1)
    return [(b0, min(n, b0 + per)) for b0 in range(0, n, per)]


def _wino_blocks(h: int, wd: int) -> bool:
    return h % 4 == 0 and (wd in (8, 16) or wd % 32 == 0)


def _wino_tiles(n: int, h: int, wd: int) -> int:
    mt = _wtile()
    return n * (-(-h // mt)) * (-(-wd // mt))


WINOGRAD_WGRAD = os.environ.get("MVAE_NO_WINOGRAD_WGRAD") is None
WINOGRAD_DY2 = os.environ.get("MVAE_NO_WINOGRAD_DY2") is None
WINOGRAD_GN = os.environ.get("MVAE_NO_WINOGRAD_GN") is None
WINOGRAD_GN_LINK = os.environ.get("MVAE_NO_WINOGRAD_GN_LINK") is None
GN_LAZY_ATTR = "_mvae_gn_lazy"
G3 = ConvGeom(3, 3, 1, 1, 1, 1, 1, False)


class LazyGn:
    __slots__ = ("x", "scale", "shift", "silu")

    def __init__(self, x, silu: bool):
        self.x, self.silu = x, int(silu)
        self.scale = self.shift = None

    def materialize(self):
        n, c, h, w = self.x.shape
        y = torch.empty_like(self.x, memory_format=CL)
        _lib.call("mvae_group_norm_apply_nhwc", self.x.data_ptr(), self.scale.data_ptr(), self.shift.data_ptr(),
                  y.data_ptr(), n, h * w, c, self.silu, 0, _stream(self.x))
        return y


class DeferredGnOutput(torch.Tensor):

    @classmethod
    def __torch_function__(cls, func, types, args=(), kwargs=None):
        if func in _DEFERRED_META:
            with torch._C.DisableTorchFunctionSubclass():
                return func(*args, **(kwargs or {}))
        name = getattr(func, "__qualname__", None) or getattr(func, "__name__", repr(func))
        raise RuntimeError(f"{name}: this GroupNorm output is deferred to its consuming convolution (the conv's Winograd "
                           "input transform applies the normalization); its values exist nowhere else. Read the conv's "
                           "output instead, or set MVAE_NO_WINOGRAD_GN=1 to have the GroupNorm write its output.")


_DEFERRED_META = {torch.Tensor.shape.__get__, torch.Tensor.size, torch.Tensor.dim, torch.Tensor.ndim.__get__,
                  torch.Tensor.data_ptr, torch.Tensor._version.__get__, torch.Tensor.is_contiguous,
                  torch.Tensor.device.__get__, torch.Tensor.dtype.__get__, torch.Tensor.is_cuda.__get__,
                  torch.Tensor.requires_grad.__get__, torch.Tensor.grad_fn.__get__, torch.Tensor.numel,
                  torch.Tensor.layout.__get__, torch.Tensor.stride, torch.Tensor.is_leaf.__get__,
                  torch.Tensor.__hash__, torch.Tensor.element_size, torch.Tensor.get_device}


def _wino_wgrad_ok(g, x, dy, dw, dys) -> bool:
    n, c, h, wd = x.shape
    co = dy.shape[1]
    return (WINOGRAD_WGRAD and _wino_ok(g, n, h, wd, c, co) and _al16(x, dy, dw) and (dys is None or _al16(dys)) and
            dy.is_contiguous(memory_format=CL) and dw.is_contiguous(memory_format=CL))


WINOGRAD_KEEP_V = os.environ.get("MVAE_NO_WINOGRAD_KEEP_V") is None


def _winograd(src, w, n: int, h: int, wd: int, k_in: int, n_out: int, src_split: bool, dgrad: bool, st, keep=None,
              gn=None, key=None, u=None, chunk=(0, 0), dkeep=None):
    mt = _wtile()
    t = _wino_tiles(n, h, wd)
    pos = (mt + 2) ** 2
    dev, kt = src.device, src if key is None else key
    if keep is not None:
        v = torch.empty(_wel() * pos * t * k_in, dtype=torch.uint8, device=dev)
        keep.append(_Kept(v, mt, kt.data_ptr(), kt._version, tuple(chunk)))
    else:
        v = ARENA.get("wino_v", _wel() * pos * t * k_in, dev)
    m = ARENA.get("wino_m", 4 * pos * t * n_out, dev)
    if u is None:
        u = ARENA.get("wino_u", _wel() * pos * k_in * n_out, dev)
        cin, cout = (n_out, k_in) if dgrad else (k_in, n_out)
        _lib.call("mvae_winograd_weight_transform", w.data_ptr(), u.data_ptr(), cin, cout, int(dgrad), mt, st)
    if dkeep is not None:
        d = torch.empty(_wel() * pos * t * k_in, dtype=torch.uint8, device=dev)
        dkeep.append(_Kept(d, mt, kt.data_ptr(), kt._version, tuple(chunk)))
        _lib.call("mvae_winograd_dy_transforms", src.data_ptr(), v.data_ptr(), d.data_ptr(), n, h, wd, k_in,
                  int(src_split), mt, st)
    elif gn is not None:
        b0 = chunk[0]
        _lib.call("mvae_winograd_input_transform_gn", src.data_ptr(), gn.scale[b0 * k_in:].data_ptr(),
                  gn.shift[b0 * k_in:].data_ptr(), gn.silu, v.data_ptr(), n, h, wd, k_in, mt, st)
    else:
        _lib.call("mvae_winograd_input_transform", src.data_ptr(), v.data_ptr(), n, h, wd, k_in, int(src_split), mt,
                  st)
    _lib.call("mvae_winograd_gemm", v.data_ptr(), u.data_ptr(), m.data_ptr(), t, k_in, n_out, mt, st)
    return m, u


BF16_DMA = os.environ.get("MVAE_NO_BF16_DMA") is None
PLANAR_DMA = os.environ.get("MVAE_PLANAR_DMA") is not None
MVAE_CONV_BF16 = 128
MVAE_CONV_PLANAR = 256


def _dma_fmt() -> int:
    if _MATH[0] == 1 and BF16_DMA:
        return 2
    if _MATH[0] == 0 and PLANAR_DMA:
        return 3
    return 0


PLANAR_MIN_MACS = 1e11


def _dma_ok(macs: float) -> bool:
    f = _dma_fmt()
    return f == 2 or (f == 3 and macs >= PLANAR_MIN_MACS)


def _dma_flag() -> int:
    return MVAE_CONV_PLANAR if _dma_fmt() == 3 else MVAE_CONV_BF16


def _dma_bytes(numel: int) -> int:
    return numel * (4 if _dma_fmt() == 3 else 2)


class _FlatWeights:
    __slots__ = ("base", "end", "buf", "fmt", "fresh", "want", "covered")

    def __init__(self):
        self.base = self.end = 0
        self.buf = None
        self.fmt = 0
        self.fresh = False
        self.want = {}
        self.covered = None


_FLATW = _FlatWeights()


class _TransposedWeights:
    __slots__ = ("slots", "want", "table", "buf", "n", "blocks", "fresh", "base", "end", "tbase", "tend", "seen",
                 "idle")

    def __init__(self):
        self.slots, self.want = {}, {}
        self.seen = set()
        self.idle = {}
        self.table = self.buf = None
        self.n = self.blocks = 0
        self.fresh = False
        self.base = self.end = self.tbase = self.tend = 0


_WT = _TransposedWeights()
BATCHED_WT = os.environ.get("MVAE_NO_BATCHED_WT") is None
WT_IDLE_STEPS = 2


def _wt_blocks(co, rs, c):
    return ((c + 63) // 64) * ((co + 63) // 64) * rs


def refresh_weight_tables(flat_data: torch.Tensor):
    n = flat_data.numel()
    _WT.base, _WT.end = flat_data.data_ptr(), flat_data.data_ptr() + 4 * n
    if BATCHED_WT:
# ... 132 lines not shown


def pack_bf16(t: torch.Tensor, key: str) -> torch.Tensor:
    out = ARENA.get(key, _dma_bytes(t.numel()), t.device)
    fn = "mvae_split_planar" if _dma_fmt() == 3 else "mvae_pack_bf16"
    _lib.call(fn, t.data_ptr(), out.data_ptr(), t.numel(), _stream(t))
    return out


_MATH = [0]


def _splits_ok() -> bool:
    return _MATH[0] != 2


class math_scope:

    def __init__(self, mode: Optional[int]):
        self.mode = mode

    def __enter__(self):
        self.prev = _MATH[0]
        if self.mode is not None and self.mode != self.prev:
            _lib.call("mvae_set_math_mode", int(self.mode))
            _MATH[0] = int(self.mode)
        return self

    def __exit__(self, *exc):
        if _MATH[0] != self.prev:
            _lib.call("mvae_set_math_mode", int(self.prev))
            _MATH[0] = self.prev
        return False


CONV_SPLITK = os.environ.get("MVAE_NO_CONV_SPLITK") is None
_CONV_WS_CACHE = {}


def _conv_call(x, w, b, res, y, n, h, wd, c, co, kh, kw, stride, pad_t, pad_l, ho, wo, mode, st):
    nbytes = 0
    if CONV_SPLITK:
        key = (n, c, co, kh, kw, ho, wo)
        nbytes = _CONV_WS_CACHE.get(key)
        if nbytes is None:
            nbytes = _CONV_WS_CACHE[key] = int(_lib.query("mvae_conv2d_split_workspace_bytes", n, c, co, kh, kw, ho, wo))
    if nbytes:
        ws = ARENA.get("convsplit", nbytes, y.device)
        _lib.call("mvae_conv2d_ws_nhwc", x, w, b, res, y.data_ptr(), n, h, wd, c, co, kh, kw, stride, pad_t, pad_l, ho,
                  wo, mode, ws.data_ptr(), ws.numel(), st)
    else:
        _lib.call("mvae_conv2d_nhwc", x, w, b, res, y.data_ptr(), n, h, wd, c, co, kh, kw, stride, pad_t, pad_l, ho, wo,
                  mode, st)


def _stride2_classes(g, h: int, wd: int) -> bool:
    return g.stride == 2 and h % 2 == 0 and wd % 2 == 0 and g.kh <= 4 and g.kw <= 4 and STRIDE2_CLASSES


@dataclass(frozen=True)
class ConvPlan:
    g: ConvGeom
    n: int
    c: int
    h: int
    w: int
    co: int
    math: int
    shape: tuple
    wino: Optional[str]
    fwd: Tuple[str, ...]
    dgrad: Tuple[str, ...]
    wgrad: Tuple[str, ...]
    tile: int
    elsize: int
    chunks: tuple
    blocks: bool
    ref: float
    dy_format: Optional[str]
    dy_bias: bool
    dy_copy_ok: bool
    dy_pack: bool
    gn_on_load: bool

    def alg(self, family: str) -> float:
        if family in ("wino", "wino_ups"):
            return self.ref * (self.tile + 2) ** 2 / (9.0 * self.tile * self.tile)
        if family in ("subpixel", "upsample"):
            return self.ref * 4 / 9
        return self.ref



def plan_conv(g: ConvGeom, n: int, c: int, h: int, w: int, cout: int, math_mode: int) -> ConvPlan:
    co, math = cout, int(math_mode)
    prev, _MATH[0] = _MATH[0], math
    try:
        ho, wo = g.out_hw(h, w)
        taps = g.kh * g.kw
        macs = float(n) * ho * wo * co * c * taps
        sub = _subpixel_upsample(g)
        s1p1 = g.kh == 3 and g.kw == 3 and g.stride == 1 and not g.upsample and \
            (g.pad_t, g.pad_l, g.pad_b, g.pad_r) == (1, 1, 1, 1)
        wino = "wino_ups" if _wino_ups_ok(g, n, h, w, c, co) else "wino" if _wino_ok(g, n, h, w, c, co) else None
        dma = _dma_ok(macs) and not g.pointwise and taps <= 32
        direct32 = _direct32(g, c, co, w)
        wino_fp32_dy = WINOGRAD_DY_FP32 and wino == "wino"
        dy_bias = bool(DYBIAS and co % 4 == 0 and ((math == 2 and wino == "wino") or wino_fp32_dy or wino == "wino_ups"))
        dy_format, copy_ok = "bias" if dy_bias else None, False
        if DYPACK and _dma_fmt() == 2 and wino != "wino" and not g.pointwise and co % 8 == 0 and taps <= 32:
            dy_format, copy_ok = "packed", not GN_BWD_FUSED and c % 8 == 0 and not g.upsample
        elif DYSPLIT and ((_dma_fmt() == 0 and math == 0) or (math == 1 and wino == "wino")) and not wino_fp32_dy and \
                not g.pointwise and not sub and co % 4 == 0 and taps <= 32 and macs >= DYSPLIT_MIN_MACS:
            dy_format, copy_ok = "split", not GN_BWD_FUSED
        dy_pack = dma and co % 8 == 0 and wino is None
        packed_dy = dy_pack or dy_format == "packed"
        pw, ups = g.pointwise, g.upsample
        def families(*rows):
            return tuple(f for f, on in rows if on)
        fwd = families((wino, wino), ("dma", dma and c % 8 == 0 and (sub or not ups)), ("pointwise", pw), ("subpixel", sub),
                       ("direct32", direct32), ("gemm", not pw and not sub))
        dgrad = families(("wino_ups", wino == "wino_ups"), ("dma", packed_dy), ("wino", wino == "wino"),
                         ("gnbwd", GN_BWD_FUSED and not pw and not ups and g.stride == 1 and co % 4 == 0),
                         ("pointwise", pw), ("upsample", ups), ("direct32", direct32),
                         ("stride2", not ups and _stride2_classes(g, h, w)), ("gemm", not pw and not ups))
        wgrad = families(("dma", packed_dy and c % 8 == 0 and not ups), ("pointwise", pw),
                         ("small_cout", SMALL_COUT_WGRAD and co <= 4 and c % 4 == 0 and s1p1),
                         ("direct", DIRECT_WGRAD and c in (32, 64) and co in DIRECT_WGRAD_COUT and math != 2 and s1p1),
                         ("wino_ups", WINOGRAD_WGRAD and wino == "wino_ups"), ("subpixel", sub),
                         ("wino", WINOGRAD_WGRAD and wino == "wino"), ("gemm", True))
        chunks = tuple(_wino_chunks(n, h, w, max(c, 4 * co if wino == "wino_ups" else co))) if wino else ()
        return ConvPlan(g, n, c, h, w, co, math, (n, c, h, w, co, g.kh, g.stride, ups), wino, fwd, dgrad, wgrad, _wtile(), _wel(), chunks, _wino_blocks(h, w),
                        2.0 * macs, dy_format, dy_bias, copy_ok, dy_pack,
                        bool(WINOGRAD_GN and WINOGRAD_WGRAD and wino == "wino"))
    finally:
        _MATH[0] = prev


def _fwd_family(p: ConvPlan, x, w, b, res, x_split, x_bf16, gn_part, lazy) -> str:
    for f in p.fwd:
        if f == "wino_ups" and (x_bf16 or x_split or lazy is not None or res is not None or gn_part is not None or
                                not _al16(x, w, b)):
            continue
        if f == "wino" and (x_bf16 or not _al16(w, b, res, lazy.x if lazy is not None else x) or
                            (gn_part is not None and not p.blocks)):
            continue
        if f == "dma" and (x_split or lazy is not None or not _al16(x)):
            continue
        if f == "direct32" and (gn_part is not None or not _al16(x, w, res)):
            continue
        return f


def _dgrad_family(p: ConvPlan, dy, w, dx, gn_link, dys, dyb) -> str:
    link = gn_link is not None and gn_link.usable(dx)
    cl, dya = dy.is_contiguous(memory_format=CL), dy if dys is None else dys
    for f in p.dgrad:
        if f == "wino_ups" and (dyb is not None or dys is not None or not cl or not _al16(dy, w)):
            continue
        if f == "dma" and (dyb is None or link):
            continue
        if f == "wino" and not (cl and _al16(dya, w)):
            continue
        if f == "gnbwd" and not (link and _al16(dy, dx)):
            continue
        if f == "direct32" and not _al16(w, dya):
            continue
        return f


def _wgrad_wino_on(p: ConvPlan) -> bool:
    return WINOGRAD_WGRAD and ("wino" in p.wgrad or "wino_ups" in p.wgrad)


def _wgrad_family(p: ConvPlan, x, dy, dw, db, x_split, dys, dyb, lazy) -> str:
    deferred = isinstance(x, DeferredGnOutput)
    cl = dy.is_contiguous(memory_format=CL) and dw.is_contiguous(memory_format=CL)
    for f in p.wgrad:
        if f == "dma" and (dyb is None or x_split or not _al16(x)):
            continue
        if f == "pointwise" and db is not None:
            continue
        if f in ("small_cout", "direct", "wino_ups", "subpixel") and deferred:
            continue
        if f == "small_cout" and not _al16(x):
            continue
        if f == "direct" and (dys is not None or not _al16(x, dy)):
            continue
        if f == "wino_ups" and (x_split or not cl or not _al16(x, dy, dw) or not _wgrad_wino_on(p)):
            continue
        if f == "wino" and not (cl and _al16(x if lazy is None else lazy.x, dy, dw, dys) and _wgrad_wino_on(p)):
            continue
        return f


class _Kept(NamedTuple):
    buf: torch.Tensor
    tile: int
    src_ptr: int
    src_version: int
    chunk: Tuple[int, int]


def _kept(entries, tile: int, src) -> dict:
    return {e.chunk: e.buf for e in entries or ()
            if e.tile == tile and e.src_ptr == src.data_ptr() and e.src_version == src._version}


def conv2d_forward_raw(x, w, b, res, g: ConvGeom, x_split: bool = False, gn_part=None, x_bf16: bool = False,
                       keep_v=None, lazy=None, plan: Optional[ConvPlan] = None):
    n, c, h, wd = x.shape
    co = w.shape[0]
    p = plan if plan is not None else plan_conv(g, n, c, h, wd, co, _MATH[0])
    ho, wo = g.out_hw(h, wd)
    y = torch.empty((n, co, ho, wo), device=x.device, dtype=torch.float32, memory_format=CL)
    st = _stream(x)
    if x_split and (g.pointwise or g.upsample or c % 4 or not _al16(x)):
# ... 17 lines not shown
                    _lib.call("mvae_winograd_output_transform_upsample", m.data_ptr(), _ptr(b), y[b0:b1].data_ptr(),
                              b1 - b0, h, wd, co, p.tile, st)
                    continue
                gp = gn_part[b0 * (h * wd // 32) * (co // 4) * 2:] if gn_part is not None else None
                _lib.call("mvae_winograd_output_transform", m.data_ptr(), _ptr(b),
                          _ptr(res[b0:b1] if res is not None else None), y[b0:b1].data_ptr(), _ptr(gp), b1 - b0, h,
                          wd, co, p.tile, st)
        return y
    dma = fam == "dma"
    if dma:
        fam = "subpixel" if g.upsample else "gemm"
    split = not dma and WEIGHT_SPLIT and _splits_ok() and c % 4 == 0 and _al16(x) and not g.pointwise and \
        g.kh * g.kw <= 32
    wfmt = _dma_fmt() if dma else int(split)
    xp = (x if x_bf16 else pack_bf16(x, "xbf")).data_ptr() if dma else x.data_ptr()
    wptr = w.data_ptr()
    if fam == "subpixel":
        wg = ARENA.get("w4", _dma_bytes(16 * co * c) if dma else 16 * co * c * 4, x.device)
        _lib.call("mvae_conv_weight_upsample_fwd", w.data_ptr(), wg.data_ptr(), co, c, wfmt, st)
        wptr = wg.data_ptr()
    elif dma or split:
        wptr = _flat_weight_ptr(w, wfmt) if wfmt != 3 else None
        if wptr is None and dma:
            wptr = pack_bf16(w, "wsplit").data_ptr()
        elif wptr is None:
            wg = ARENA.get("wsplit", w.numel() * 4, x.device)
            _lib.call("mvae_split_bf16", w.data_ptr(), wg.data_ptr(), w.numel(), st)
            wptr = wg.data_ptr()
    with _timed("conv_fwd", p.alg(fam), p.shape, p.ref):
        if fam == "pointwise":
            _lib.call("mvae_gemm_strided_batched", 0, 1, n * h * wd, co, c, 1.0, xp, c, 0,
                      wptr, c, 0, 0.0, y.data_ptr(), co, 0, 1, _ptr(b), _ptr(res), co, 0, None, 0, st)
        elif fam == "subpixel":
            _lib.call("mvae_conv2d_upsample_nhwc", xp, wptr, _ptr(b), _ptr(res), y.data_ptr(), n, h, wd, c, co, wfmt, st)
        elif fam == "direct32":
            _lib.call("mvae_conv2d_direct32_nhwc", xp, wptr, _ptr(b), _ptr(res), y.data_ptr(), n, h, wd,
                      (MVAE_CONV_WSPLIT if split else 0) | (MVAE_CONV_XSPLIT if x_split else 0), st)
        else:
            mode = _dma_flag() if dma else \
                (1 if g.upsample else 0) | (MVAE_CONV_WSPLIT if split else 0) | (MVAE_CONV_XSPLIT if x_split else 0)
            if gn_part is not None:
                _lib.call("mvae_conv2d_gnstats_nhwc", xp, wptr, _ptr(b), _ptr(res), y.data_ptr(),
                          n, h, wd, c, co, g.kh, g.kw, g.stride, g.pad_t, g.pad_l, ho, wo, mode, gn_part.data_ptr(), st)
            else:
                _conv_call(xp, wptr, _ptr(b), _ptr(res), y, n, h, wd, c, co, g.kh, g.kw, g.stride, g.pad_t, g.pad_l,
                           ho, wo, mode, st)
    return y


def _in_hw(g: ConvGeom, ho: int, wo: int) -> Tuple[int, int]:
    return (ho // 2, wo // 2) if g.upsample else \
        ((ho - 1) * g.stride + g.kh - g.pad_t - g.pad_b, (wo - 1) * g.stride + g.kw - g.pad_l - g.pad_r)


def pack_dy(dy: torch.Tensor, g: ConvGeom, cin: int, bias_out=None, beta: float = 1.0, plan: Optional[ConvPlan] = None):
    if dy.dim() != 4 or not _al16(dy) or not dy.is_contiguous(memory_format=CL):
        return None, False
    n, co, ho, wo = dy.shape
    if plan is None:
        plan = plan_conv(g, n, cin, *_in_hw(g, ho, wo), co, _MATH[0])
    if not plan.dy_pack:
        return None, False
    if bias_out is None:
        return pack_bf16(dy, "dybf"), False
    rows = n * ho * wo
    out = ARENA.get("dybf", _dma_bytes(dy.numel()), dy.device)
    ws = ARENA.get("bias", _lib.query("mvae_bias_grad_workspace_bytes", rows, co), dy.device)
    fn = "mvae_split_planar_colsum" if _dma_fmt() == 3 else "mvae_pack_bf16_colsum"
    _lib.call(fn, dy.data_ptr(), out.data_ptr(), rows, co, bias_out.data_ptr(), float(beta), ws.data_ptr(), ws.numel(),
              _stream(dy))
    return out, True


def split_dy(dy: torch.Tensor) -> Optional[torch.Tensor]:
    if not DY_SPLIT or not _splits_ok() or dy.dim() != 4 or dy.shape[1] % 4 or dy.numel() < DY_SPLIT_MIN or not _al16(dy) or \
            not dy.is_contiguous(memory_format=CL):
        return None
    ds = torch.empty_like(dy, memory_format=CL)
    _lib.call("mvae_split_bf16", dy.data_ptr(), ds.data_ptr(), dy.numel(), _stream(dy))
    return ds


def conv2d_dgrad_raw(dy, w, x_shape, g: ConvGeom, gn_link=None, dys=None, dyb=None, dkeep=None, out=None,
                     beta: float = 0.0, plan: Optional[ConvPlan] = None):
    n, c, h, wd = x_shape
    co = w.shape[0]
    _, _, ho, wo = dy.shape
    p = plan if plan is not None else plan_conv(g, n, c, h, wd, co, _MATH[0])
    if out is not None and not g.pointwise:
        raise RuntimeError("conv2d_dgrad_raw: an accumulating output is for 1x1 convs")
    dx = out if out is not None else torch.empty((n, c, h, wd), device=dy.device, dtype=torch.float32,
                                                 memory_format=CL)
    st = _stream(dy)
    if dys is not None and (g.pointwise or co % 4):
        dys = None
    dya = dy if dys is None else dys
    fam = _dgrad_family(p, dy, w, dx, gn_link, dys, dyb)
    mt, pos = p.tile, (p.tile + 2) ** 2
    dma = fam == "dma"
    if dma:
        fam, dya = "upsample" if g.upsample else "stride2" if "stride2" in p.dgrad else "gemm", dyb
    split = not dma and WEIGHT_SPLIT and _splits_ok() and \
        (fam == "gnbwd" or (co % 4 == 0 and _al16(dy) and g.kh * g.kw <= 32))
    wfmt, wbytes = (_dma_fmt(), _dma_bytes) if dma else (int(split), lambda numel: 4 * numel)
    cflag = _dma_flag() if dma else (MVAE_CONV_WSPLIT if split else 0) | (MVAE_CONV_XSPLIT if dys is not None else 0)
    kflag = (8 if wfmt == 3 else 4) if dma else int(split) | (2 if dys is not None else 0)
    if fam == "upsample":
        wt = ARENA.get("wt", wbytes(c * 16 * co), dy.device)
        _lib.call("mvae_conv_weight_upsample_dgrad", w.data_ptr(), wt.data_ptr(), co, c, wfmt, st)
    elif fam in ("gnbwd", "stride2", "gemm"):
        wtp = _weight_t(w, co, g.kh, g.kw, c, wfmt, wbytes(c * g.kh * g.kw * co), st)
    with _timed("conv_dgrad", p.alg(fam), p.shape, p.ref):
        if fam == "wino_ups":
            kc = ARENA.get("wups_k", 4 * co * 9 * c * 4, dy.device)
            _lib.call("mvae_winograd_upsample_weights", w.data_ptr(), kc.data_ptr(), c, co, st)
            u = ARENA.get("wino_u", p.elsize * pos * c * 4 * co, dy.device)
            _lib.call("mvae_winograd_weight_transform", kc.data_ptr(), u.data_ptr(), c, 4 * co, 1, mt, st)
            for b0, b1 in p.chunks:
                nb, t = b1 - b0, _wino_tiles(b1 - b0, h, wd)
                v = ARENA.get("wino_v", p.elsize * pos * t * 4 * co, dy.device)
                if dkeep is not None:
                    d = torch.empty(p.elsize * pos * t * 4 * co, dtype=torch.uint8, device=dy.device)
                    dkeep.append(_Kept(d, mt, dy.data_ptr(), dy._version, (b0, b1)))
                else:
                    d = ARENA.get("wino_d", p.elsize * pos * t * 4 * co, dy.device)
                _lib.call("mvae_winograd_dy_transforms_upsample", dy[b0:b1].data_ptr(), v.data_ptr(), d.data_ptr(), nb,
                          h, wd, co, mt, st)
                m = ARENA.get("wino_m", 4 * pos * t * c, dy.device)
                _lib.call("mvae_winograd_gemm", v.data_ptr(), u.data_ptr(), m.data_ptr(), t, 4 * co, c, mt, st)
                _lib.call("mvae_winograd_output_transform", m.data_ptr(), None, None, dx[b0:b1].data_ptr(), None, nb, h,
                          wd, c, mt, st)
        elif fam == "wino":
            L = gn_link if gn_link is not None and gn_link.usable(dx) and p.blocks else None
            part = torch.empty(n * h * wd // 32 * c * 2, device=dy.device, dtype=torch.float64) if L else None
            u = None
            for b0, b1 in p.chunks:
                nb = b1 - b0
                m, u = _winograd(dya[b0:b1], w, nb, h, wd, co, c, dys is not None, True, st, u=u, key=dya,
                                 chunk=(b0, b1), dkeep=dkeep)
                if L is None:
                    _lib.call("mvae_winograd_output_transform", m.data_ptr(), None, None, dx[b0:b1].data_ptr(), None, nb,
                              h, wd, c, mt, st)
                else:
                    _lib.call("mvae_winograd_output_gnbwd", m.data_ptr(), dx[b0:b1].data_ptr(), L.x[b0:b1].data_ptr(),
                              L.mean[b0 * L.groups:].data_ptr(), L.rstd[b0 * L.groups:].data_ptr(),
                              L.gamma.data_ptr(), L.beta.data_ptr(), L.groups, L.silu,
                              part[b0 * (h * wd // 32) * c * 2:].data_ptr(), nb, h, wd, c, mt, st)
            if L is not None:
                L.part, L.dx = part, dx
        elif fam == "gnbwd":
            L = gn_link
            part = torch.empty(n * h * wd // 32 * c * 2, device=dy.device, dtype=torch.float64)
            _lib.call("mvae_conv2d_dgrad_gnbwd_nhwc", dya.data_ptr(), wtp, dx.data_ptr(), n, ho, wo, co, c,
                      g.kh, g.kw, g.pad_t, g.pad_l, h, wd, kflag, L.x.data_ptr(), L.mean.data_ptr(),
                      L.rstd.data_ptr(), L.gamma.data_ptr(), L.beta.data_ptr(), L.groups, L.silu, part.data_ptr(), st)
            L.part, L.dx = part, dx
        elif fam == "pointwise":
            _lib.call("mvae_gemm_strided_batched", 0, 0, n * h * wd, c, co, 1.0, dy.data_ptr(), co, 0, w.data_ptr(), c,
                      0, float(beta), dx.data_ptr(), c, 0, 1, None, None, 0, 0, None, 0, st)
        elif fam == "upsample":
            _lib.call("mvae_conv2d_nhwc", dya.data_ptr(), wt.data_ptr(), None, None, dx.data_ptr(), n, ho, wo, co, c,
                      4, 4, 2, 1, 1, h, wd, cflag, st)
        elif fam == "direct32":
            _lib.call("mvae_conv2d_direct32_nhwc", dya.data_ptr(), w.data_ptr(), None, None, dx.data_ptr(), n, h, wd,
                      MVAE_CONV_DGRAD_DIRECT | (MVAE_CONV_XSPLIT if dys is not None else 0), st)
        elif fam == "stride2":
            wc = ARENA.get("wcls", c * g.kh * g.kw * co * 4, dy.device)
            _lib.call("mvae_conv2d_dgrad_stride2_nhwc", dya.data_ptr(), wtp, dx.data_ptr(), n, h, wd, c, co,
                      g.kh, g.kw, g.pad_t, g.pad_l, ho, wo, kflag, wc.data_ptr(), wc.numel(), st)
        else:
            _conv_call(dya.data_ptr(), wtp, None, None, dx, n, ho, wo, co, c, g.kh, g.kw, g.stride, g.pad_t,
                       g.pad_l, h, wd, 2 | cflag, st)
    return dx


def conv2d_wgrad_raw(dy, x, dw, beta: float, g: ConvGeom, db=None, x_split: bool = False, dys=None, dyb=None,
                     x_bf16: bool = False, wino_v=None, wino_d=None, lazy=None, plan: Optional[ConvPlan] = None):
    n, c, h, wd = x.shape
    _, co, ho, wo = dy.shape
    p = plan if plan is not None else plan_conv(g, n, c, h, wd, co, _MATH[0])
    fam = _wgrad_family(p, x, dy, dw, db, x_split, dys, dyb, lazy)
    if lazy is not None and fam != "wino":
        x, lazy = lazy.materialize(), None
        fam = _wgrad_family(p, x, dy, dw, db, x_split, dys, dyb, None)
    if x_bf16 and fam != "dma":
        raise RuntimeError("conv2d wgrad: a packed bf16 input needs the bf16-mixed LDS-DMA path (packed dy, cout % 8)")
    if isinstance(x, DeferredGnOutput) and (lazy is None or fam != "wino"):
        raise RuntimeError("conv2d wgrad: a deferred GroupNorm output reached a weight-gradient kernel that reads x")
    if x_split and (g.pointwise or g.upsample):
        raise RuntimeError("conv2d wgrad: a pre-split input needs a non-pointwise, non-upsample conv")
    st, dev = _stream(dy), dy.device
    mt, pos = p.tile, (p.tile + 2) ** 2

    def ws(query, *args):
        return ARENA.get("ws", _lib.query(query, *args), dev)

    with _timed("conv_wgrad", p.alg(fam), p.shape, p.ref):
        if fam == "pointwise":
            m = n * h * wd
            s = ws("mvae_gemm_workspace_bytes", co, c, m, 1)
            _lib.call("mvae_gemm_strided_batched", 1, 0, co, c, m, 1.0, dy.data_ptr(), co, 0, x.data_ptr(), c, 0,
                      float(beta), dw.data_ptr(), c, 0, 1, None, None, 0, 0, s.data_ptr(), s.numel(), st)
            return False
        if fam in ("small_cout", "direct", "subpixel"):
            fn = {"small_cout": "mvae_conv2d_wgrad_small_cout", "direct": "mvae_conv2d_wgrad_direct",
                  "subpixel": "mvae_conv2d_wgrad_upsample"}[fam]
            s = ws(fn + "_workspace_bytes", *((n, c) if fam == "small_cout" else (n, h, wd, c, co)))
            _lib.call(fn + "_nhwc", dy.data_ptr(), x.data_ptr(), dw.data_ptr(), _ptr(db), float(beta), n, h, wd, c, co,
                      *(() if fam == "subpixel" else (int(x_split),)), s.data_ptr(), s.numel(), st)
            return db is not None
        if fam == "wino_ups":
            kept, kept_d = _kept(wino_v, mt, x), _kept(wino_d, mt, dy)
            dkc = ARENA.get("wups_dk", 4 * co * 9 * c * 4, dev)
            for i, (b0, b1) in enumerate(p.chunks):
                nb, t = b1 - b0, _wino_tiles(b1 - b0, h, wd)
                v, dt = kept.get((b0, b1)), kept_d.get((b0, b1))
                if dt is None:
                    dt = ARENA.get("wino_d", p.elsize * pos * t * 4 * co, dev)
                    _lib.call("mvae_winograd_dy_transforms_upsample", dy[b0:b1].data_ptr(), None, dt.data_ptr(), nb, h,
                              wd, co, mt, st)
                if v is None:
                    v = ARENA.get("wino_v", p.elsize * pos * t * c, dev)
                    _lib.call("mvae_winograd_input_transform", x[b0:b1].data_ptr(), v.data_ptr(), nb, h, wd, c, 0, mt,
                              st)
                m = ARENA.get("wino_mw", 4 * pos * 4 * co * c, dev)
                s = ws("mvae_gemm_workspace_bytes", 4 * co, c, t, pos)
                _lib.call("mvae_winograd_wgrad_gemm", dt.data_ptr(), v.data_ptr(), m.data_ptr(), t, 4 * co, c, mt,
                          s.data_ptr(), s.numel(), st)
                _lib.call("mvae_winograd_wgrad_output", m.data_ptr(), dkc.data_ptr(), 0.0 if i == 0 else 1.0, 4 * co, c,
                          mt, st)
            _lib.call("mvae_winograd_upsample_fold", dkc.data_ptr(), dw.data_ptr(), float(beta), c, co, st)
            return False
        if fam == "wino":
            dya = dys if dys is not None else dy
            kept, kept_d = _kept(wino_v, mt, x), _kept(wino_d, mt, dya)
            for i, (b0, b1) in enumerate(p.chunks):
                nb, t = b1 - b0, _wino_tiles(b1 - b0, h, wd)
                v, dt = kept.get((b0, b1)), kept_d.get((b0, b1))
                m = ARENA.get("wino_mw", 4 * pos * co * c, dev)
                s = ws("mvae_gemm_workspace_bytes", co, c, t, pos)
                if dt is None:
                    dt = ARENA.get("wino_d", p.elsize * pos * t * co, dev)
                    _lib.call("mvae_winograd_dy_transform", dya[b0:b1].data_ptr(), dt.data_ptr(), nb, h, wd, co,
                              int(dys is not None), mt, st)
                if v is None and lazy is not None:
                    v = ARENA.get("wino_v", p.elsize * pos * t * c, dev)
                    _lib.call("mvae_winograd_input_transform_gn", lazy.x[b0:b1].data_ptr(),
                              lazy.scale[b0 * c:].data_ptr(), lazy.shift[b0 * c:].data_ptr(), lazy.silu, v.data_ptr(),
                              nb, h, wd, c, mt, st)
                elif v is None:
                    v = ARENA.get("wino_v", p.elsize * pos * t * c, dev)
                    _lib.call("mvae_winograd_input_transform", x[b0:b1].data_ptr(), v.data_ptr(), nb, h, wd, c,
                              int(x_split), mt, st)
                _lib.call("mvae_winograd_wgrad_gemm", dt.data_ptr(), v.data_ptr(), m.data_ptr(), t, co, c, mt,
                          s.data_ptr(), s.numel(), st)
                _lib.call("mvae_winograd_wgrad_output", m.data_ptr(), dw.data_ptr(), float(beta) if i == 0 else 1.0, co,
                          c, mt, st)
            return False
        dya, xp, mode = dy, x, (1 if g.upsample else 0) | (MVAE_CONV_XSPLIT if x_split else 0)
        if fam == "dma":
            dya, xp, mode, db = dyb, x if x_bf16 else pack_bf16(x, "xbf"), _dma_flag(), None
        elif dys is not None and co % 4 == 0:
            dya, mode, db = dys, mode | MVAE_CONV_DYSPLIT, None
        s = ws("mvae_conv2d_wgrad_workspace_bytes", n, c, co, g.kh, g.kw, ho, wo)
        _lib.call("mvae_conv2d_wgrad_nhwc", dya.data_ptr(), xp.data_ptr(), dw.data_ptr(), _ptr(db), float(beta), n, h, wd,
                  c, co, g.kh, g.kw, g.stride, g.pad_t, g.pad_l, ho, wo, mode, s.data_ptr(), s.numel(), st)
        return db is not None


def bias_grad_raw(dy2d_ptr, rows, n, out, beta, device, stream):
    nbytes = _lib.query("mvae_bias_grad_workspace_bytes", rows, n)
    ws = ARENA.get("bias", nbytes, device)
    _lib.call("mvae_bias_grad", dy2d_ptr, rows, n, n, out.data_ptr(), float(beta), ws.data_ptr(), ws.numel(), stream)


class DxSum:
    __slots__ = ("n", "left", "buf")

    def __init__(self, n: int):
        self.n = self.left = n
        self.buf = None


DX_SUM = os.environ.get("MVAE_NO_DX_SUM") is None


class GradSink:
    __slots__ = ("g", "closed")

    def __init__(self):
        self.g = None
        self.closed = False

    def park(self, g) -> bool:
        if self.closed:
            return False
        self.g = g
        return True

    def take(self):
        g, self.g = self.g, None
        self.closed = g is None
        return g


DYPACK_ATTR = "_mvae_dypack"
DYPACK = os.environ.get("MVAE_NO_DYPACK") is None
DYSPLIT = os.environ.get("MVAE_NO_DYSPLIT") is None
DYBIAS = os.environ.get("MVAE_NO_DYBIAS") is None
WINOGRAD_DY_FP32 = os.environ.get("MVAE_WINOGRAD_DY_SPLIT") is None
DYSPLIT_MIN_MACS = 1e11


class DyPack:
    __slots__ = ("bias_ref", "packed", "dx_ref", "dx_version", "dx_shape", "bias_done", "db", "fmt", "nodx",
                 "copy_ok")

    def __init__(self, bias_ref, fmt: str = "packed", copy_ok: bool = False):
        self.bias_ref = bias_ref
        self.fmt = fmt
        self.packed = self.dx_ref = self.dx_version = self.dx_shape = self.db = None
        self.bias_done = False
        self.nodx = False
        self.copy_ok = copy_ok

    def take(self, dy):
        packed, ref, ver, shp, nodx = self.packed, self.dx_ref, self.dx_version, self.dx_shape, self.nodx
        out = (packed, self.bias_done, self.db)
        self.packed = self.dx_ref = self.dx_version = self.dx_shape = self.db = None
        self.bias_done = self.nodx = False
        dx = ref() if ref is not None else None
        if packed is None or dx is None or dy.data_ptr() != dx.data_ptr() or dy._version != ver or \
                tuple(dy.shape) != shp or not dy.is_contiguous(memory_format=CL):
            if nodx:
                raise RuntimeError("conv2d backward: the GroupNorm wrote only the copy of its dx for this conv (its only "
                                   "consumer), but the conv's output gradient is another tensor")
            return None
        return out


BWD_OVERLAP = os.environ.get("MVAE_BWD_OVERLAP", "1") != "0"
BWD_OVERLAP_MAX_FLOPS = float(os.environ.get("MVAE_BWD_OVERLAP_MAX_GF", "200")) * 1e9
_SIDE = {}


def _bwd_side(t: torch.Tensor):
    if not BWD_OVERLAP or PROFILE is not None or not t.is_cuda:
        return None
    side = _SIDE.get(t.device)
    if side is None:
        if torch.cuda.is_current_stream_capturing():
            return None
        side = _SIDE[t.device] = (torch.cuda.Stream(t.device), torch.cuda.Event(), torch.cuda.Event())
        _SIDE_STREAMS.add(side[0].cuda_stream)
    return side


class Conv2dFn(torch.autograd.Function):
    @staticmethod
    def forward(ctx, x, weight, bias, residual, geom: ConvGeom, res_sink=None, x_sink=None, gn_part=None,
                gn_link=None, dypack=None, grad_on: bool = True, dx_sum=None, plan: Optional[ConvPlan] = None):
        _check(x, "conv input")
        xs = bool(getattr(x, XSPLIT_ATTR, False))
        xb16 = bool(getattr(x, BF16_ATTR, False))
        lazy = getattr(x, GN_LAZY_ATTR, None)
        if (xs or xb16) and not x.is_contiguous(memory_format=CL):
            raise RuntimeError("conv2d: a pre-split / packed input must not be re-laid out")
        w = _krsc(weight)
        res = nhwc(residual) if residual is not None else None
        want_w = bool(weight.requires_grad and grad_on)
        if plan is None:
            plan = plan_conv(geom, *x.shape, w.shape[0], _MATH[0])
        if lazy is not None and not (_fwd_family(plan, x, w, bias, res, xs, xb16, gn_part, lazy) == "wino" and
                                     (not want_w or "wino" in plan.wgrad)):
            x, lazy = lazy.materialize(), None
        if lazy is None:
            x = nhwc(x)
        keep = [] if (WINOGRAD_KEEP_V or lazy is not None) and want_w else None
        y = conv2d_forward_raw(x, w, bias, res, geom, xs, gn_part, x_bf16=xb16, keep_v=keep, lazy=lazy, plan=plan)
        ctx.wino_v = keep if keep else None
        ctx.lazy = lazy
        ctx.math = plan.math
        ctx.geom, ctx.plan = geom, plan
        ctx.x_split = xs
        ctx.x_bf16 = xb16
        ctx.has_bias = bias is not None
        ctx.has_res = residual is not None
        ctx.save_for_backward(x, w)
        ctx.weight_ref = weight
        ctx.bias_ref = bias
        ctx.res_sink, ctx.x_sink = res_sink, x_sink
        ctx.gn_link = gn_link
        ctx.dx_sum = dx_sum
        ctx.dypack = dypack
        return y

    @staticmethod
    def backward(ctx, dy):
        with math_scope(ctx.math):
            return Conv2dFn._backward(ctx, dy)

    @staticmethod
    def _backward(ctx, dy):
        x, w = ctx.saved_tensors
        g, plan = ctx.geom, ctx.plan
        dy = nhwc(dy)
        dx = dw_ret = db_ret = dres = None
        link = ctx.gn_link
        if link is not None:
            link.part = link.dx = None
        want_b = ctx.has_bias and ctx.needs_input_grad[2]
        bias_done = False
        dyb = None
        got = ctx.dypack.take(dy) if ctx.dypack is not None else None
        dys = None
        if got is not None:
            taken, bias_done, db_ret = got
            if ctx.dypack.fmt == "packed":
                dyb = taken
            elif ctx.dypack.fmt == "split":
                dys = taken
            if not want_b:
                db_ret = None
            elif bias_done:
                bt = _main_grad(ctx.bias_ref)
                if bt is not None:
                    bt.add_(db_ret)
                    db_ret = None
        elif ctx.needs_input_grad[0] or ctx.needs_input_grad[1]:
            bt = _main_grad(ctx.bias_ref) if want_b else None
            if want_b and bt is None:
                db_ret = torch.empty(dy.shape[1], device=dy.device, dtype=torch.float32)
            dyb, bias_done = pack_dy(dy, g, w.shape[1], bt if bt is not None else db_ret, 1.0 if bt is not None else 0.0,
                                     plan)
            if not bias_done:
                db_ret = None
        if dys is None and not g.pointwise and not _subpixel_upsample(g) and dyb is None:
            dys = split_dy(dy)
        dkeep = None

        def wgrad():
            nonlocal dw_ret, bias_done
            tgt = _main_grad(ctx.weight_ref)
            if tgt is None:
                dw_ret = torch.empty_like(w, memory_format=CL)
            btgt = _main_grad(ctx.bias_ref) if tgt is not None and want_b and not bias_done else None
            fused = conv2d_wgrad_raw(dy, x, dw_ret if tgt is None else tgt, 0.0 if tgt is None else 1.0, g, btgt,
                                     x_split=ctx.x_split, dys=dys, dyb=dyb, x_bf16=ctx.x_bf16, wino_v=ctx.wino_v,
                                     wino_d=dkeep, lazy=ctx.lazy, plan=plan)
            bias_done = bias_done or fused

        side = _bwd_side(dy) if ctx.needs_input_grad[0] and ctx.needs_input_grad[1] and \
            _main_grad(ctx.weight_ref) is not None and not g.pointwise and min(plan.c, plan.co) >= 32 and \
            plan.ref <= BWD_OVERLAP_MAX_FLOPS else None
        if side is not None:
            stream, ev_fork, ev_join = side
            main = torch.cuda.current_stream(dy.device)
            ev_fork.record(main)
            stream.wait_event(ev_fork)
            with torch.cuda.stream(stream):
                wgrad()
            ev_join.record(stream)
        dkeep = [] if (WINOGRAD_DY2 and side is None and dyb is None and ctx.needs_input_grad[0] and
                       ctx.needs_input_grad[1] and _wgrad_wino_on(plan)) else None
        acc = ctx.dx_sum
        if ctx.needs_input_grad[0] and acc is not None:
            if not _al16(dy):
                dy = dy.clone(memory_format=CL)
            first = acc.buf is None
            if first:
                acc.buf = torch.empty(tuple(x.shape), device=dy.device, dtype=torch.float32, memory_format=CL)
            conv2d_dgrad_raw(dy, w, x.shape, g, out=acc.buf, beta=0.0 if first else 1.0, plan=plan)
            acc.left -= 1
            dx = None
            if acc.left == 0:
                dx, acc.buf, acc.left = acc.buf, None, acc.n
        elif ctx.needs_input_grad[0]:
            dx = conv2d_dgrad_raw(dy, w, x.shape, g, link if ctx.x_sink is None else None, dys=dys, dyb=dyb,
                                  dkeep=dkeep, plan=plan)
            if ctx.x_sink is not None and ctx.x_sink.park(dx):
                dx = None
        if side is not None:
            main.wait_event(ev_join)
        elif ctx.needs_input_grad[1]:
            wgrad()
        ctx.wino_v = dkeep = None
        if ctx.has_bias and ctx.needs_input_grad[2] and not bias_done:
            tgt = _main_grad(ctx.bias_ref)
            n, co, ho, wo = dy.shape
            if tgt is not None:
                bias_grad_raw(dy.data_ptr(), n * ho * wo, co, tgt, 1.0, dy.device, _stream(dy))
            else:
                db_ret = torch.empty(co, device=dy.device, dtype=torch.float32)
                bias_grad_raw(dy.data_ptr(), n * ho * wo, co, db_ret, 0.0, dy.device, _stream(dy))
        if ctx.has_res and ctx.needs_input_grad[3]:
            dres = dy
            if ctx.res_sink is not None and ctx.res_sink.park(dy):
                dres = None
        if ctx.needs_input_grad[1] and dw_ret is None:
            _grad_done(ctx.weight_ref)
        if want_b and db_ret is None:
            _grad_done(ctx.bias_ref)
        return dx, dw_ret, db_ret, dres, None, None, None, None, None, None, None, None, None


GN_PART_ATTR = "_mvae_gn_part"
GN_FUSED_STATS = os.environ.get("MVAE_NO_GN_FUSED") is None and os.environ.get("MVAE_NO_VEC_EPI") is None


def conv2d(x, weight, bias, geom: ConvGeom, residual=None, res_sink=None, x_sink=None, gn_stats: bool = False,
           gn_bias: bool = False, dx_sum=None):
    n, c, h, w = x.shape
    co = weight.shape[0]
    plan = plan_conv(geom, n, c, h, w, co, _MATH[0])
    part = None
    if gn_stats and GN_FUSED_STATS and not geom.pointwise and not _subpixel_upsample(geom) and c % 4 == 0:
        ho, wo = geom.out_hw(h, w)
        if (ho * wo) % 32 == 0 and co % 4 == 0 and _al16(x, weight, bias, residual):
            part = torch.empty(n * ho * wo // 32 * (co // 4) * 2, device=x.device, dtype=torch.float64)
    link = getattr(x, GN_BWD_ATTR, None)
    if link is not None and not link.matches(x):
        link = None
    fmt = plan.dy_format if gn_stats else "bias" if gn_bias and plan.dy_bias else None
    if fmt == "bias" and not (bias is not None and bias.requires_grad):
        fmt = None
    dyp = DyPack(bias, fmt, plan.dy_copy_ok and fmt == plan.dy_format) if fmt and torch.is_grad_enabled() else None
    if dx_sum is not None and not (DX_SUM and geom.pointwise and torch.is_grad_enabled() and x_sink is None):
        dx_sum = None
    y = Conv2dFn.apply(x, weight, bias, residual, geom, res_sink, x_sink, part, link, dyp, torch.is_grad_enabled(),
                       dx_sum, plan)
    if part is not None:
        setattr(y, GN_PART_ATTR, (part, y._version))
    if dyp is not None:
        setattr(y, DYPACK_ATTR, (dyp, y._version))
    return y


GN_BWD_ATTR = "_mvae_gn_bwd_link"
GN_BWD_FUSED = os.environ.get("MVAE_GN_BWD_FUSED") is not None and os.environ.get("MVAE_NO_VEC_EPI") is None


class GnBwdLink:
    __slots__ = ("x", "gamma", "beta", "mean", "rstd", "groups", "silu", "y_ref", "y_version", "part", "dx")

    def __init__(self, groups: int, silu: bool):
        self.groups, self.silu = groups, int(silu)
        self.x = self.gamma = self.beta = self.mean = self.rstd = None
        self.y_ref = self.y_version = self.part = self.dx = None

    def bind_output(self, y):
        self.y_ref, self.y_version = y.data_ptr(), y._version

    def matches(self, x) -> bool:
        return self.x is not None and x.data_ptr() == self.y_ref and x._version == self.y_version

    def usable(self, dx) -> bool:
        n, c, h, w = dx.shape
        return (self.x is not None and tuple(self.x.shape) == (n, c, h, w) and (h * w) % 32 == 0 and
                c % self.groups == 0 and (c // self.groups) % 4 == 0 and _al16(self.x))

    def take(self, dy):
        part, dx = self.part, self.dx
        self.part = self.dx = None
        if part is None or dx is None or dy.data_ptr() != dx.data_ptr() or dy.shape != dx.shape or \
                not dy.is_contiguous(memory_format=CL):
            return None
        return part


class GroupNormFn(torch.autograd.Function):
    @staticmethod
    def forward(ctx, x, gamma, beta, groups: int, eps: float, silu: bool, drop_p: float, seed: int,
                y_split: bool = False, grad_sink=None, part=None, link=None, dypack=None, lazy=None,
                conv_dy_only: bool = False):
        _check(x, "group_norm input")
        x = nhwc(x)
        n, c, h, w = x.shape
        mean = torch.empty(n * groups, device=x.device, dtype=torch.float32)
        rstd = torch.empty_like(mean)
        nbytes = _lib.query("mvae_group_norm_workspace_bytes", n, h * w, c)
        ws = ARENA.get("gn", nbytes, x.device)
        if lazy is not None:
            lazy.x = x
            lazy.scale = torch.empty(n * c, device=x.device, dtype=torch.float32)
            lazy.shift = torch.empty_like(lazy.scale)
            with _timed("gn_fwd", 0.0 if part is not None else 4.0 * x.numel(), (n, c, h * w)):
                _lib.call("mvae_group_norm_stats_nhwc", x.data_ptr(), _ptr(part), gamma.data_ptr(), beta.data_ptr(),
                          mean.data_ptr(), rstd.data_ptr(), lazy.scale.data_ptr(), lazy.shift.data_ptr(), n, h * w, c,
                          groups, float(eps), ws.data_ptr(), ws.numel(), _stream(x))
            y = torch.full((1,), float("nan"), device=x.device).expand(n, c, h, w)
        else:
            y = torch.empty_like(x, memory_format=CL)
            with _timed("gn_fwd", 8.0 * x.numel(), (n, c, h * w)):
                if part is not None:
                    _lib.call("mvae_group_norm_fwd_part_nhwc", x.data_ptr(), part.data_ptr(), gamma.data_ptr(),
                              beta.data_ptr(), y.data_ptr(), mean.data_ptr(), rstd.data_ptr(), n, h * w, c, groups,
                              float(eps), int(silu), float(drop_p), int(seed) & 0xFFFFFFFFFFFFFFFF, int(y_split),
                              ws.data_ptr(), ws.numel(), _stream(x))
                else:
                    _lib.call("mvae_group_norm_fwd_nhwc", x.data_ptr(), gamma.data_ptr(), beta.data_ptr(),
                              y.data_ptr(), mean.data_ptr(), rstd.data_ptr(), n, h * w, c, groups, float(eps),
                              int(silu), float(drop_p), int(seed) & 0xFFFFFFFFFFFFFFFF, int(y_split), ws.data_ptr(),
                              ws.numel(), _stream(x))
        ctx.save_for_backward(x, gamma, beta, mean, rstd)
        ctx.cfg = (groups, int(silu), float(drop_p), int(seed) & 0xFFFFFFFFFFFFFFFF)
        ctx.gamma_ref, ctx.beta_ref = gamma, beta
        ctx.grad_sink = grad_sink
        ctx.link = link
        ctx.dypack = dypack
        ctx.conv_dy_only = conv_dy_only
        if link is not None:
            link.x, link.gamma, link.beta, link.mean, link.rstd = x, gamma, beta, mean, rstd
        return y

    @staticmethod
    def backward(ctx, dy):
        x, gamma, beta, mean, rstd = ctx.saved_tensors
        groups, silu, drop_p, seed = ctx.cfg
        dy = nhwc(dy)
        n, c, h, w = x.shape
        dx = torch.empty_like(x, memory_format=CL)
        dg_ret = db_ret = None
        dg = _main_grad(ctx.gamma_ref) if ctx.needs_input_grad[1] else None
        db = _main_grad(ctx.beta_ref) if ctx.needs_input_grad[2] else None
        if ctx.needs_input_grad[1] and dg is None:
            dg = dg_ret = torch.zeros(c, device=x.device, dtype=torch.float32)
        if ctx.needs_input_grad[2] and db is None:
            db = db_ret = torch.zeros(c, device=x.device, dtype=torch.float32)
        nbytes = _lib.query("mvae_group_norm_workspace_bytes", n, h * w, c)
        ws = ARENA.get("gn", nbytes, x.device)
        add = ctx.grad_sink.take() if ctx.grad_sink is not None else None
        if add is not None:
            add = nhwc(add)
            if add.shape != x.shape or add.dtype != torch.float32:
                raise RuntimeError("group_norm backward: parked branch gradient has the wrong shape")
        gpart = ctx.link.take(dy) if ctx.link is not None and drop_p == 0.0 else None
        req = ctx.dypack if ctx.dypack is not None and _al16(dy, dx) and (add is None or _al16(add)) else None
        if req is not None and gpart is not None and req.fmt == "packed":
            req = None
        bias_only = req is not None and req.fmt == "bias"
        if bias_only and not (req.bias_ref is not None and req.bias_ref.requires_grad):
            req = None
        packed = tgt = cs = None
        if bias_only and req is not None:
            tgt = req.db = torch.empty(c, device=x.device, dtype=torch.float32)
            csb = _lib.query("mvae_group_norm_colsum_workspace_bytes", n, h * w, c)
            cs = ARENA.get("gncs", csb, x.device)
            packed = True
        elif req is not None:
            packed = (torch.empty_like(x, memory_format=CL) if req.fmt == "split" else
                      torch.empty(x.numel() * 2, device=x.device, dtype=torch.uint8))
            bref = req.bias_ref
            if bref is not None and bref.requires_grad:
                tgt = req.db = torch.empty(c, device=x.device, dtype=torch.float32)
            csb = _lib.query("mvae_group_norm_colsum_workspace_bytes", n, h * w, c)
            cs = ARENA.get("gncs", csb, x.device) if tgt is not None else None
        nodx = bool(ctx.conv_dy_only and DX_COPY_ONLY and req is not None and not bias_only and req.copy_ok)
        dxp = None if nodx else dx.data_ptr()
        if nodx and DX_POISON:
            dx.fill_(float("nan"))
        with _timed("gn_bwd", (12.0 + (4.0 if add is not None else 0.0)) * x.numel(), (n, c, h * w)):
            if gpart is not None and req is not None:
                _lib.call("mvae_group_norm_bwd_part_split_nhwc", x.data_ptr(), dy.data_ptr(), gpart.data_ptr(),
                          gamma.data_ptr(), beta.data_ptr(), mean.data_ptr(), rstd.data_ptr(), dxp,
                          _ptr(add), _ptr(dg), _ptr(db), n, h * w, c, groups, silu, ws.data_ptr(), ws.numel(),
                          None if bias_only else packed.data_ptr(), _ptr(tgt), 0.0, _ptr(cs),
                          cs.numel() if cs is not None else 0, _stream(x))
            elif gpart is not None:
                _lib.call("mvae_group_norm_bwd_part_nhwc", x.data_ptr(), dy.data_ptr(), gpart.data_ptr(),
                          gamma.data_ptr(), beta.data_ptr(), mean.data_ptr(), rstd.data_ptr(), dx.data_ptr(),
                          _ptr(add), _ptr(dg), _ptr(db), n, h * w, c, groups, silu, ws.data_ptr(), ws.numel(),
                          _stream(x))
            elif bias_only and req is not None:
                _lib.call("mvae_group_norm_bwd_colsum_nhwc", x.data_ptr(), dy.data_ptr(), gamma.data_ptr(),
                          beta.data_ptr(), mean.data_ptr(), rstd.data_ptr(), dx.data_ptr(), _ptr(add), _ptr(dg),
                          _ptr(db), n, h * w, c, groups, silu, drop_p, seed, ws.data_ptr(), ws.numel(), tgt.data_ptr(),
                          0.0, cs.data_ptr(), cs.numel(), _stream(x))
            elif req is not None:
                _lib.call("mvae_group_norm_bwd_split_nhwc" if req.fmt == "split" else "mvae_group_norm_bwd_pack_nhwc",
                          x.data_ptr(), dy.data_ptr(), gamma.data_ptr(),
                          beta.data_ptr(), mean.data_ptr(), rstd.data_ptr(), dxp, _ptr(add), _ptr(dg),
                          _ptr(db), n, h * w, c, groups, silu, drop_p, seed, ws.data_ptr(), ws.numel(),
                          packed.data_ptr(), _ptr(tgt), 0.0, _ptr(cs), cs.numel() if cs is not None else 0,
                          _stream(x))
            else:
                _lib.call("mvae_group_norm_bwd_nhwc", x.data_ptr(), dy.data_ptr(), gamma.data_ptr(), beta.data_ptr(),
                          mean.data_ptr(), rstd.data_ptr(), dx.data_ptr(), _ptr(add), _ptr(dg), _ptr(db), n, h * w,
                          c, groups, silu, drop_p, seed, ws.data_ptr(), ws.numel(), _stream(x))
        if req is not None:
            req.packed, req.dx_ref, req.dx_version, req.dx_shape = packed, weakref.ref(dx), dx._version, \
                tuple(dx.shape)
            req.bias_done = tgt is not None
            req.nodx = nodx
        if ctx.needs_input_grad[1] and dg_ret is None:
            _grad_done(ctx.gamma_ref)
        if ctx.needs_input_grad[2] and db_ret is None:
            _grad_done(ctx.beta_ref)
        return dx, dg_ret, db_ret, None, None, None, None, None, None, None, None, None, None, None, None


XSPLIT_ATTR = "_mvae_xsplit"
ACT_SPLIT = os.environ.get("MVAE_NO_ACT_SPLIT") is None
BF16_ATTR = "_mvae_bf16"


DX_COPY_ONLY = os.environ.get("MVAE_NO_DX_COPY_ONLY") is None
DX_POISON = os.environ.get("MVAE_DX_POISON") == "1"


def group_norm(x, gamma, beta, groups, eps=1e-6, silu=False, drop_p=0.0, seed=0, for_conv=False, grad_sink=None,
               conv_dy_only: bool = False):
    plan = plan_conv(G3, *x.shape, int(for_conv), _MATH[0]) if for_conv and not isinstance(for_conv, bool) else None
    packed = plan is not None and plan.fwd[0] == "dma" and plan.co % 8 == 0 and _al16(x)
    split = _dma_fmt() if packed else int(bool(for_conv and ACT_SPLIT and _splits_ok() and _dma_fmt() == 0 and
                                                x.shape[1] % 4 == 0))
    part = getattr(x, GN_PART_ATTR, None)
    if part is not None:
        delattr(x, GN_PART_ATTR)
        h, w = x.shape[2], x.shape[3]
        ok = part[1] == x._version and (h * w) % 32 == 0 and (x.shape[1] // groups) % 4 == 0 and \
            x.shape[1] % groups == 0 and x.is_contiguous(memory_format=CL)
        part = part[0] if ok else None
    link = GnBwdLink(groups, silu) if (for_conv and GN_BWD_FUSED and drop_p == 0.0 and x.requires_grad) else None
    dyp = getattr(x, DYPACK_ATTR, None)
    if dyp is not None:
        delattr(x, DYPACK_ATTR)
        dyp = dyp[0] if dyp[1] == x._version and x.is_contiguous(memory_format=CL) and _al16(x) else None
    lazy = None
    if plan is not None and plan.gn_on_load and drop_p == 0.0 and _al16(x):
        n, c, h, w = x.shape
        lazy, split = LazyGn(x, silu), 0
        if (link is None and WINOGRAD_GN_LINK and x.requires_grad and dyp is not None and dyp.fmt != "packed" and
                plan.blocks and c % groups == 0 and (c // groups) % 4 == 0 and
                _lib.query("mvae_group_norm_bwd_streaming", n, h * w, c, groups, 1)):
            link = GnBwdLink(groups, silu)
    y = GroupNormFn.apply(x, gamma, beta, groups, eps, silu, drop_p, seed, split, grad_sink, part, link, dyp, lazy,
                          conv_dy_only)
    if lazy is not None:
        y = y.as_subclass(DeferredGnOutput)
        setattr(y, GN_LAZY_ATTR, lazy)
# ... 935 lines not shown
```

Before: 791.1 images/s.

## Defer GroupNorm input gradient into the following conv's Winograd dy transform

```diff
diff --git a/include/medvae_hip.h b/include/medvae_hip.h
--- a/include/medvae_hip.h
+++ b/include/medvae_hip.h
@@ -84,6 +84,13 @@
                                void* stream);
 int mvae_winograd_dy_transforms(const float* dy, void* v, void* d, int nb, int h, int w, int k, int dy_split, int tile,
                                 void* stream);
+int mvae_group_norm_bwd_dy_rows(int nb, int h, int w, int k, int tile);
+int mvae_group_norm_bwd_dy_transforms(const float* x, const float* dy, const float* coef, long long coef_stride,
+                                      int img0, int silu, void* v, void* d, float* colsum, int nb, int h, int w, int k,
+                                      int tile, void* stream);
+size_t mvae_group_norm_bwd_dy_bias_workspace_bytes(int k);
+int mvae_group_norm_bwd_dy_bias(const float* colsum, long long rows, int k, float* dbias, float beta, void* workspace,
+                                size_t workspace_bytes, void* stream);
 int mvae_winograd_wgrad_gemm(const void* d, const void* v, float* m, long long tiles, int cout, int cin, int tile,
                              float* workspace, size_t workspace_bytes, void* stream);
 int mvae_winograd_wgrad_output(const float* m, float* dw, float beta, int cout, int cin, int tile, void* stream);
@@ -186,6 +193,9 @@
                                         int groups, int silu, void* workspace, size_t workspace_bytes, void* dx_split,
                                         float* dbias, float bias_beta, void* cs_workspace, size_t cs_workspace_bytes,
                                         void* stream);
+int mvae_group_norm_bwd_part_coef_nhwc(const double* part, const float* gamma, const float* beta, const float* mean,
+                                       const float* rstd, float* dgamma, float* dbeta, int nb, int hw, int c,
+                                       int groups, void* workspace, size_t workspace_bytes, float* coef, void* stream);
 int mvae_group_norm_bwd_streaming(int nb, int hw, int c, int groups, int with_dxp);
 int mvae_group_norm_fwd_part_nhwc(const float* x, const double* part, const float* gamma, const float* beta, float* y,
                                   float* mean, float* rstd, int nb, int hw, int c, int groups, float eps, int silu,
diff --git a/medvae_disentangled_multimodal_amd/_lib.py b/medvae_disentangled_multimodal_amd/_lib.py
--- a/medvae_disentangled_multimodal_amd/_lib.py
+++ b/medvae_disentangled_multimodal_amd/_lib.py
@@ -37,6 +37,11 @@
     "mvae_winograd_output_gnbwd": (I, [P, P, P, P, P, P, P, I, I, P, I, I, I, I, I, P]),
     "mvae_winograd_dy_transform": (I, [P, P, I, I, I, I, I, I, P]),
     "mvae_winograd_dy_transforms": (I, [P, P, P, I, I, I, I, I, I, P]),
+    "mvae_group_norm_bwd_dy_rows": (I, [I, I, I, I, I]),
+    "mvae_group_norm_bwd_dy_transforms": (I, [P, P, P, L, I, I, P, P, P, I, I, I, I, I, P]),
+    "mvae_group_norm_bwd_dy_bias_workspace_bytes": (Z, [I]),
+    "mvae_group_norm_bwd_dy_bias": (I, [P, L, I, P, F, P, Z, P]),
+    "mvae_group_norm_bwd_part_coef_nhwc": (I, [P, P, P, P, P, P, P, I, I, I, I, P, Z, P, P]),
     "mvae_winograd_wgrad_gemm": (I, [P, P, P, L, I, I, I, P, Z, P]),
     "mvae_winograd_wgrad_output": (I, [P, P, F, I, I, I, P]),
     "mvae_winograd_upsample_weights": (I, [P, P, I, I, P]),
diff --git a/medvae_disentangled_multimodal_amd/csrc/norm.hip b/medvae_disentangled_multimodal_amd/csrc/norm.hip
--- a/medvae_disentangled_multimodal_amd/csrc/norm.hip
+++ b/medvae_disentangled_multimodal_amd/csrc/norm.hip
@@ -299,6 +299,20 @@
     k2[i] = (float)(-rs * rs * A2 / n);
     k3[i] = (float)(-rs * A1 / n + mu * rs * rs * A2 / n);
   }
+}
+
+__global__ void __launch_bounds__(256) gn_bwd_coef_kernel(GnArgs a, const float* __restrict__ k1,
+                                                          const float* __restrict__ k2, const float* __restrict__ k3,
+                                                          float* __restrict__ coef, long long stride) {
+  const long long i = (long long)blockIdx.x * 256 + threadIdx.x;
+  if (i >= (long long)a.nb * a.C) return;
+  const int b = (int)(i / a.C), c = (int)(i - (long long)b * a.C), bg = b * a.G + c / (a.C / a.G);
+  const float sc = a.rstd[bg] * a.gamma[c];
+  coef[i] = sc;
+  coef[stride + i] = a.beta[c] - a.mean[bg] * sc;
+  coef[2 * stride + i] = k1[i];
+  coef[3 * stride + i] = k2[bg];
+  coef[4 * stride + i] = k3[bg];
 }
 
 constexpr int GN_PG_SLICES = 64;
@@ -1320,7 +1334,7 @@
                        const float* mean, const float* rstd, float* dx, const float* dx_add, float* dgamma,
                        float* dbeta, int nb, int hw, int c, int groups, int silu, void* workspace,
                        size_t workspace_bytes, void* dx_split, float* dbias, float bias_beta, void* cs_ws,
-                       void* stream);
+                       void* stream, float* coef = nullptr);
 
 int mvae_group_norm_bwd_part_nhwc(const float* x, const float* dy, const double* part, const float* gamma,
                                   const float* beta, const float* mean, const float* rstd, float* dx,
@@ -1368,12 +1382,12 @@
                        const float* mean, const float* rstd, float* dx, const float* dx_add, float* dgamma,
                        float* dbeta, int nb, int hw, int c, int groups, int silu, void* workspace,
                        size_t workspace_bytes, void* dx_split, float* dbias, float bias_beta, void* cs_ws,
-                       void* stream) {
+                       void* stream, float* coef) {
   if (nb <= 0 || hw <= 0 || c <= 0 || (c & 3) || groups <= 0 || c % groups || hw % 32 || part == nullptr) {
     set_error("group_norm_bwd_part: needs hw %% 32 == 0 and C %% 4 == 0");
     return MVAE_EINVAL;
   }
-  if (dx == nullptr && dx_split == nullptr) {
+  if (dx == nullptr && dx_split == nullptr && coef == nullptr) {
     set_error("group_norm_bwd_part: dx may be null only when the split copy is written");
     return MVAE_EINVAL;
   }
@@ -1405,11 +1419,28 @@
     hipLaunchKernelGGL(gn_param_final_kernel, dim3(cdiv(c, 256)), dim3(256), 0, st, c, (const double*)pg, dgamma,
                        dbeta);
   }
+  if (coef) {
+    hipLaunchKernelGGL(gn_bwd_coef_kernel, dim3(cdiv((long long)nb * c, 256)), dim3(256), 0, st, a, k1, k2, k3, coef,
+                       (long long)nb * c);
+    return launch_status();
+  }
   hipLaunchKernelGGL(gn_dx_kernel, dim3(a.chunks, nb), dim3(256), 0, st, a, k1, k2, k3, dx);
   if (dbias)
     hipLaunchKernelGGL(gn_colsum_final_kernel, dim3(cdiv(c, 16)), dim3(256), 0, st, (const double*)a.csp,
                        nb * a.chunks, c, dbias, bias_beta);
   return launch_status();
+}
+
+int mvae_group_norm_bwd_part_coef_nhwc(const double* part, const float* gamma, const float* beta, const float* mean,
+                                       const float* rstd, float* dgamma, float* dbeta, int nb, int hw, int c,
+                                       int groups, void* workspace, size_t workspace_bytes, float* coef,
+                                       void* stream) {
+  if (coef == nullptr || ((uintptr_t)coef & 15)) {
+    set_error("group_norm_bwd_part_coef: 16-B aligned coefficient rows");
+    return MVAE_EINVAL;
+  }
+  return gn_bwd_part(nullptr, nullptr, part, gamma, beta, mean, rstd, nullptr, nullptr, dgamma, dbeta, nb, hw, c, groups,
+                     0, workspace, workspace_bytes, nullptr, nullptr, 0.f, nullptr, stream, coef);
 }
 
 }
diff --git a/medvae_disentangled_multimodal_amd/csrc/winograd.hip b/medvae_disentangled_multimodal_amd/csrc/winograd.hip
--- a/medvae_disentangled_multimodal_amd/csrc/winograd.hip
+++ b/medvae_disentangled_multimodal_amd/csrc/winograd.hip
@@ -452,6 +452,11 @@
   }
 }
 
+template <int MT>
+__device__ __forceinline__ long long wino_tiles_dev(int nb, int H, int W) {
+  return (long long)nb * ((H + MT - 1) / MT) * ((W + MT - 1) / MT);
+}
+
 template <bool UPS>
 struct DySrc {
   unsigned pix0, chan, rowb;
@@ -510,14 +515,20 @@
     for (int j = 0; j < AL; ++j) wstore_f<SF>(vr, base + (unsigned)(i * AL + j) * plane, o[i][j]);
 }
 
-template <int MT, bool XS, int SF = 0, bool UPS = false>
-__global__ void __launch_bounds__(256) wino_dy2_kernel(const float* __restrict__ dy, uint4* __restrict__ v,
-                                                       uint4* __restrict__ d, int nb, int H, int W, int K) {
+struct WinoGnb {
+  const float* x;
+  const float* coef;
+  long long stride;
+  float* colsum;
+};
+
+template <int MT, bool XS, int SF, bool UPS, int GNB>
+__device__ __forceinline__ float4 wino_dy2_tile(const float* __restrict__ dy, uint4* __restrict__ v,
+                                                uint4* __restrict__ d, int nb, int H, int W, int K, long long idx,
+                                                const WinoGnb& gb) {
   constexpr int AL = MT + 2;
   const int K4 = K >> 2, th = (H + MT - 1) / MT, tw = (W + MT - 1) / MT;
   const long long T = (long long)nb * th * tw;
-  const long long idx = (long long)blockIdx.x * blockDim.x + threadIdx.x;
-  if (idx >= T * K4) return;
   const long long t = idx / K4;
   const int k4 = (int)(idx - t * K4);
   const int tj = (int)(t % tw), ti = (int)((t / tw) % th), b = (int)(t / ((long long)tw * th));
@@ -536,6 +547,52 @@
       const float4 r = bload4(xr, ok ? src.off(h, w) : OOB);
       p[i][j] = XS ? split4_to_f32(r) : r;
     }
+  float4 bsum{0.f, 0.f, 0.f, 0.f};
+  if constexpr (GNB != 0) {
+    const __amdgpu_buffer_rsrc_t gr = make_rsrc(gb.x, (unsigned)((long long)nb * H * W * K * 4));
+    const float* cf = gb.coef + (long long)b * K + k4 * 4;
+    const float4 sc = *(const float4*)cf, sh = *(const float4*)(cf + gb.stride);
+    const float4 cp = *(const float4*)(cf + 2 * gb.stride), cq = *(const float4*)(cf + 3 * gb.stride);
+    const float4 cr = *(const float4*)(cf + 4 * gb.stride);
+    const float c1[4] = {sc.x, sc.y, sc.z, sc.w}, c2[4] = {sh.x, sh.y, sh.z, sh.w}, c3[4] = {cp.x, cp.y, cp.z, cp.w};
+    const float c4[4] = {cq.x, cq.y, cq.z, cq.w}, c5[4] = {cr.x, cr.y, cr.z, cr.w};
+#pragma unroll
+    for (int i0 = 0; i0 < AL; i0 += 2) {
+      float4 xv[2][AL];
+#pragma unroll
+      for (int i = 0; i < 2; ++i)
+#pragma unroll
+        for (int j = 0; j < AL; ++j) {
+          const int h = MT * ti - 1 + i0 + i, w = MT * tj - 1 + j;
+          const bool ok = (unsigned)h < (unsigned)H && (unsigned)w < (unsigned)W;
+          xv[i][j] = bload4(gr, ok ? src.off(h, w) : OOB);
+        }
+#pragma unroll
+      for (int i = 0; i < 2; ++i)
+#pragma unroll
+        for (int j = 0; j < AL; ++j) {
+          const int h = MT * ti - 1 + i0 + i, w = MT * tj - 1 + j;
+          const bool ok = (unsigned)h < (unsigned)H && (unsigned)w < (unsigned)W;
+          const float xs[4] = {xv[i][j].x, xv[i][j].y, xv[i][j].z, xv[i][j].w};
+          const float4 g = p[i0 + i][j];
+          float o[4] = {g.x, g.y, g.z, g.w};
+#pragma unroll
+          for (int e = 0; e < 4; ++e) {
+            if constexpr (GNB == 2) {
+              const float a = fmaf(xs[e], c1[e], c2[e]);
+              const float s = __builtin_amdgcn_rcpf(1.f + __expf(-a));
+              o[e] = o[e] * (s * fmaf(a, 1.f - s, 1.f));
+            }
+            o[e] = fmaf(c3[e], o[e], fmaf(c4[e], xs[e], c5[e]));
+          }
+          p[i0 + i][j] = ok ? float4{o[0], o[1], o[2], o[3]} : float4{0.f, 0.f, 0.f, 0.f};
+        }
+    }
+#pragma unroll
+    for (int u = 0; u < MT; ++u)
+#pragma unroll
+      for (int e = 0; e < MT; ++e) bsum = f4add(bsum, p[1 + u][1 + e]);
+  }
 #pragma unroll
   for (int i = 0; i < AL; ++i) {
     float4 ci[MT], o[AL];
@@ -565,6 +622,32 @@
   for (int i = 0; i < AL; ++i)
 #pragma unroll
     for (int j = 0; j < AL; ++j) wstore_f<SF>(vr, base + (unsigned)(i * AL + j) * plane, p[i][j]);
+  return bsum;
+}
+
+template <int MT, bool XS, int SF = 0, bool UPS = false>
+__global__ void __launch_bounds__(256) wino_dy2_kernel(const float* __restrict__ dy, uint4* __restrict__ v,
+                                                       uint4* __restrict__ d, int nb, int H, int W, int K) {
+  const long long idx = (long long)blockIdx.x * blockDim.x + threadIdx.x;
+  if (idx >= wino_tiles_dev<MT>(nb, H, W) * (K >> 2)) return;
+  wino_dy2_tile<MT, XS, SF, UPS, 0>(dy, v, d, nb, H, W, K, idx, WinoGnb{});
+}
+
+template <int MT, int SF, int GNB>
+__global__ void __launch_bounds__(256) wino_dy2_gnb_kernel(const float* __restrict__ dy, uint4* __restrict__ v,
+                                                           uint4* __restrict__ d, int nb, int H, int W, int K,
+                                                           WinoGnb gb) {
+  __shared__ float4 red[256];
+  const int tid = threadIdx.x, K4 = K >> 2;
+  const long long idx = (long long)blockIdx.x * blockDim.x + tid;
+  float4 bs{0.f, 0.f, 0.f, 0.f};
+  if (idx < wino_tiles_dev<MT>(nb, H, W) * K4) bs = wino_dy2_tile<MT, false, SF, false, GNB>(dy, v, d, nb, H, W, K, idx, gb);
+  red[tid] = bs;
+  __syncthreads();
+  if (tid < K4) {
+    for (int q = tid + K4; q < 256; q += K4) bs = f4add(bs, red[q]);
+    *(float4*)(gb.colsum + (long long)blockIdx.x * K + tid * 4) = bs;
+  }
 }
 
 __host__ __device__ constexpr int ups_tap(int p, int r) { return p == 0 ? (r == 0 ? 0 : 1) : (r == 2 ? 2 : 1); }
@@ -774,6 +857,43 @@
   }
   if (both) hipLaunchKernelGGL((wino_dy2_kernel<MT, false, SF>), g, dim3(256), 0, st, dy, vv, dd, nb, h, w, k);
   else hipLaunchKernelGGL((wino_dy_kernel<MT, false, SF>), g, dim3(256), 0, st, dy, dd, nb, h, w, k);
+}
+
+static long long dy_gnb_rows(int nb, int h, int w, int k, int mt) {
+  const int k4 = k / 4;
+  return (k4 > 0 && k4 <= 256 && 256 % k4 == 0) ? (wino_tiles(nb, h, w, mt) * k4 + 255) / 256 : 0;
+}
+
+template <int MT, int SF>
+static void dy_gnb_go(const float* dy, void* v, void* d, int nb, int h, int w, int k, int silu, WinoGnb gb,
+                      hipStream_t st) {
+  const dim3 g((unsigned)dy_gnb_rows(nb, h, w, k, MT));
+  if (silu) hipLaunchKernelGGL((wino_dy2_gnb_kernel<MT, SF, 2>), g, dim3(256), 0, st, dy, (uint4*)v, (uint4*)d, nb, h, w, k, gb);
+  else hipLaunchKernelGGL((wino_dy2_gnb_kernel<MT, SF, 1>), g, dim3(256), 0, st, dy, (uint4*)v, (uint4*)d, nb, h, w, k, gb);
+}
+
+constexpr int WCS_SLICES = 64;
+__global__ void __launch_bounds__(256) wino_colsum_slice_kernel(const float* __restrict__ part, long long rows, int K,
+                                                                double* __restrict__ sl_out) {
+  __shared__ double sh[256];
+  const int cl = threadIdx.x & 63, rg = threadIdx.x >> 6;
+  const int c = blockIdx.x * 64 + cl, sl = blockIdx.y;
+  const long long lo = rows * sl / WCS_SLICES, hi = rows * (sl + 1) / WCS_SLICES;
+  double s = 0.0;
+  if (c < K)
+    for (long long i = lo + rg; i < hi; i += 4) s += (double)part[i * K + c];
+  sh[threadIdx.x] = s;
+  __syncthreads();
+  if (rg == 0 && c < K) sl_out[(long long)sl * K + c] = sh[cl] + sh[cl + 64] + sh[cl + 128] + sh[cl + 192];
+}
+
+__global__ void __launch_bounds__(256) wino_colsum_final_kernel(const double* __restrict__ sl_in, int K,
+                                                                float* __restrict__ out, float beta) {
+  const int c = blockIdx.x * 256 + threadIdx.x;
+  if (c >= K) return;
+  double s = 0.0;
+  for (int sl = 0; sl < WCS_SLICES; ++sl) s += sl_in[(long long)sl * K + c];
+  out[c] = (beta != 0.f ? beta * out[c] : 0.f) + (float)s;
 }
 
 template <int MT, int WSEG>
@@ -992,6 +1112,45 @@
   return launch_status();
 }
 
+int mvae_group_norm_bwd_dy_rows(int nb, int h, int w, int k, int tile) {
+  return (tile == 4 && wino_sf() == 0 && wino_geom_ok(tile, nb, h, w, k, k)) ? (int)dy_gnb_rows(nb, h, w, k, tile) : 0;
+}
+
+int mvae_group_norm_bwd_dy_transforms(const float* x, const float* dy, const float* coef, long long coef_stride,
+                                      int img0, int silu, void* v, void* d, float* colsum, int nb, int h, int w, int k,
+                                      int tile, void* stream) {
+  if (!x || !dy || !coef || !v || !d || !colsum || img0 < 0 || coef_stride < (long long)(img0 + nb) * k ||
+      coef_stride % 4 || !al16(x) || !al16(dy) || !al16(coef) || !al16(v) || !al16(d) || !al16(colsum) ||
+      mvae_group_norm_bwd_dy_rows(nb, h, w, k, tile) <= 0) {
+    set_error("group_norm_bwd_dy_transforms: the 3xBF16 arithmetic, tile 4, k / 4 a divisor of 256, 16-B aligned, "
+              "coefficient rows covering the images");
+    return MVAE_EINVAL;
+  }
+  const WinoGnb gb{x, coef + (long long)img0 * k, coef_stride, colsum};
+  dy_gnb_go<4, 0>(dy, v, d, nb, h, w, k, silu, gb, (hipStream_t)stream);
+  return launch_status();
+}
+
+size_t mvae_group_norm_bwd_dy_bias_workspace_bytes(int k) { return (size_t)WCS_SLICES * std::max(k, 0) * sizeof(double); }
+
+int mvae_group_norm_bwd_dy_bias(const float* colsum, long long rows, int k, float* dbias, float beta, void* workspace,
+                                size_t workspace_bytes, void* stream) {
+  if (!colsum || !dbias || !workspace || rows <= 0 || k <= 0 || ((uintptr_t)workspace & 7)) {
+    set_error("group_norm_bwd_dy_bias: partial rows, a bias gradient and an 8-B aligned workspace");
+    return MVAE_EINVAL;
+  }
+  if (workspace_bytes < mvae_group_norm_bwd_dy_bias_workspace_bytes(k)) {
+    set_error("group_norm_bwd_dy_bias: workspace too small");
+    return MVAE_EWORKSPACE;
+  }
+  hipStream_t st = (hipStream_t)stream;
+  hipLaunchKernelGGL(wino_colsum_slice_kernel, dim3(cdiv(k, 64), WCS_SLICES), dim3(256), 0, st, colsum, rows, k,
+                     (double*)workspace);
+  hipLaunchKernelGGL(wino_colsum_final_kernel, dim3(cdiv(k, 256)), dim3(256), 0, st, (const double*)workspace, k, dbias,
+                     beta);
+  return launch_status();
+}
+
 int mvae_winograd_wgrad_gemm(const void* d, const void* v, float* m, long long tiles, int cout, int cin, int tile,
                              float* workspace, size_t workspace_bytes, void* stream) {
   if (!d || !v || !m || tiles <= 0 || cout <= 0 || cin <= 0 || cout % 4 || cin % 4 || !al16(d) || !al16(v) || !al16(m) ||
diff --git a/medvae_disentangled_multimodal_amd/ops.py b/medvae_disentangled_multimodal_amd/ops.py
--- a/medvae_disentangled_multimodal_amd/ops.py
+++ b/medvae_disentangled_multimodal_amd/ops.py
@@ -279,15 +279,56 @@
 
 class DeferredGnOutput(torch.Tensor):
 
+    _READ_MSG = ("this GroupNorm output is deferred to its consuming convolution (the conv's Winograd input transform "
+                 "applies the normalization); its values exist nowhere else. Read the conv's output instead, or set "
+                 "MVAE_NO_WINOGRAD_GN=1 to have the GroupNorm write its output.")
+
     @classmethod
     def __torch_function__(cls, func, types, args=(), kwargs=None):
         if func in _DEFERRED_META:
             with torch._C.DisableTorchFunctionSubclass():
                 return func(*args, **(kwargs or {}))
         name = getattr(func, "__qualname__", None) or getattr(func, "__name__", repr(func))
-        raise RuntimeError(f"{name}: this GroupNorm output is deferred to its consuming convolution (the conv's Winograd "
-                           "input transform applies the normalization); its values exist nowhere else. Read the conv's "
-                           "output instead, or set MVAE_NO_WINOGRAD_GN=1 to have the GroupNorm write its output.")
+        raise RuntimeError(f"{name}: {cls._READ_MSG}")
+
+
+WINOGRAD_GNBWD_LOAD = os.environ.get("MVAE_NO_WINOGRAD_GNBWD_LOAD") is None
+GNB_LAZY_ATTR = "_mvae_gnb_lazy"
+
+
+class LazyGnGrad:
+    __slots__ = ("x", "dy", "coef", "silu", "part", "gamma", "beta", "mean", "rstd", "groups", "colsum")
+
+    def __init__(self, x, dy, coef, silu, part, gamma, beta, mean, rstd, groups):
+        self.x, self.dy, self.coef, self.silu, self.part = x, dy, coef, int(silu), part
+        self.gamma, self.beta, self.mean, self.rstd, self.groups = gamma, beta, mean, rstd, groups
+        self.colsum = None
+
+    def materialize(self):
+        x = self.x
+        n, c, h, w = x.shape
+        dx = torch.empty_like(x, memory_format=CL)
+        db = torch.empty(c, device=x.device, dtype=torch.float32)
+        ws = ARENA.get("gn", _lib.query("mvae_group_norm_workspace_bytes", n, h * w, c), x.device)
+        cs = ARENA.get("gncs", _lib.query("mvae_group_norm_colsum_workspace_bytes", n, h * w, c), x.device)
+        _lib.call("mvae_group_norm_bwd_part_split_nhwc", x.data_ptr(), self.dy.data_ptr(), self.part.data_ptr(),
+                  self.gamma.data_ptr(), self.beta.data_ptr(), self.mean.data_ptr(), self.rstd.data_ptr(),
+                  dx.data_ptr(), None, None, None, n, h * w, c, self.groups, self.silu, ws.data_ptr(), ws.numel(), None,
+                  db.data_ptr(), 0.0, cs.data_ptr(), cs.numel(), _stream(x))
+        return dx, db
+
+
+class DeferredGnGrad(DeferredGnOutput):
+    _READ_MSG = ("this GroupNorm input gradient is deferred to the backward of the convolution that produced the "
+                 "GroupNorm's input (its Winograd dy transform computes it on load); its values exist nowhere else. Set "
+                 "MVAE_NO_WINOGRAD_GNBWD_LOAD=1 to have the GroupNorm backward write it.")
+
+
+def _engine_runs(node) -> bool:
+    try:
+        return node is not None and bool(torch._C._will_engine_execute_node(node))
+    except Exception:
+        return False
 
 
 _DEFERRED_META = {torch.Tensor.shape.__get__, torch.Tensor.size, torch.Tensor.dim, torch.Tensor.ndim.__get__,
@@ -309,7 +350,7 @@
 
 
 def _winograd(src, w, n: int, h: int, wd: int, k_in: int, n_out: int, src_split: bool, dgrad: bool, st, keep=None,
-              gn=None, key=None, u=None, chunk=(0, 0), dkeep=None):
+              gn=None, key=None, u=None, chunk=(0, 0), dkeep=None, gnb=None):
     mt = _wtile()
     t = _wino_tiles(n, h, wd)
     pos = (mt + 2) ** 2
@@ -327,8 +368,15 @@
     if dkeep is not None:
         d = torch.empty(_wel() * pos * t * k_in, dtype=torch.uint8, device=dev)
         dkeep.append(_Kept(d, mt, kt.data_ptr(), kt._version, tuple(chunk)))
-        _lib.call("mvae_winograd_dy_transforms", src.data_ptr(), v.data_ptr(), d.data_ptr(), n, h, wd, k_in,
-                  int(src_split), mt, st)
+        if gnb is not None:
+            rec, cs = gnb
+            b0 = chunk[0]
+            _lib.call("mvae_group_norm_bwd_dy_transforms", rec.x[b0:b0 + n].data_ptr(), rec.dy[b0:b0 + n].data_ptr(),
+                      rec.coef.data_ptr(), rec.coef.numel() // 5, b0, rec.silu, v.data_ptr(), d.data_ptr(),
+                      cs.data_ptr(), n, h, wd, k_in, mt, st)
+        else:
+            _lib.call("mvae_winograd_dy_transforms", src.data_ptr(), v.data_ptr(), d.data_ptr(), n, h, wd, k_in,
+                      int(src_split), mt, st)
     elif gn is not None:
         b0 = chunk[0]
         _lib.call("mvae_winograd_input_transform_gn", src.data_ptr(), gn.scale[b0 * k_in:].data_ptr(),
@@ -627,6 +675,7 @@
     dy_copy_ok: bool
     dy_pack: bool
     gn_on_load: bool
+    gnb_on_load: bool = False
 
     def alg(self, family: str) -> float:
         if family in ("wino", "wino_ups"):
@@ -677,7 +726,10 @@
         chunks = tuple(_wino_chunks(n, h, w, max(c, 4 * co if wino == "wino_ups" else co))) if wino else ()
         return ConvPlan(g, n, c, h, w, co, math, (n, c, h, w, co, g.kh, g.stride, ups), wino, fwd, dgrad, wgrad, _wtile(), _wel(), chunks, _wino_blocks(h, w),
                         2.0 * macs, dy_format, dy_bias, copy_ok, dy_pack,
-                        bool(WINOGRAD_GN and WINOGRAD_WGRAD and wino == "wino"))
+                        bool(WINOGRAD_GN and WINOGRAD_WGRAD and wino == "wino"),
+                        bool(WINOGRAD_GNBWD_LOAD and WINOGRAD_DY2 and math == 0 and _wtile() == 4 and
+                             dgrad[:1] == ("wino",) and wgrad[:1] == ("wino",) and dy_format == "bias" and
+                             co % 4 == 0 and 256 % (co // 4) == 0))
     finally:
         _MATH[0] = prev
 
@@ -861,7 +913,7 @@
 
 
 def conv2d_dgrad_raw(dy, w, x_shape, g: ConvGeom, gn_link=None, dys=None, dyb=None, dkeep=None, out=None,
-                     beta: float = 0.0, plan: Optional[ConvPlan] = None):
+                     beta: float = 0.0, plan: Optional[ConvPlan] = None, gnb=None):
     n, c, h, wd = x_shape
     co = w.shape[0]
     _, _, ho, wo = dy.shape
@@ -875,6 +927,8 @@
         dys = None
     dya = dy if dys is None else dys
     fam = _dgrad_family(p, dy, w, dx, gn_link, dys, dyb)
+    if gnb is not None and fam != "wino":
+        raise RuntimeError("conv2d dgrad: a deferred GroupNorm input gradient reached a kernel that reads dy")
     mt, pos = p.tile, (p.tile + 2) ** 2
     dma = fam == "dma"
     if dma:
@@ -913,10 +967,17 @@
             L = gn_link if gn_link is not None and gn_link.usable(dx) and p.blocks else None
             part = torch.empty(n * h * wd // 32 * c * 2, device=dy.device, dtype=torch.float64) if L else None
             u = None
-            for b0, b1 in p.chunks:
+            if gnb is not None:
+                rows = [_lib.query("mvae_group_norm_bwd_dy_rows", b1 - b0, h, wd, co, mt) for b0, b1 in p.chunks]
+                if dkeep is None or dys is not None or min(rows) <= 0:
+                    raise RuntimeError("conv2d dgrad: no one-pass dy transform for a deferred GroupNorm input gradient")
+                cs = ARENA.get("wino_cs", 4 * sum(rows) * co, dy.device)
+                gnb.colsum = (cs, sum(rows))
+            for i, (b0, b1) in enumerate(p.chunks):
                 nb = b1 - b0
                 m, u = _winograd(dya[b0:b1], w, nb, h, wd, co, c, dys is not None, True, st, u=u, key=dya,
-                                 chunk=(b0, b1), dkeep=dkeep)
+                                 chunk=(b0, b1), dkeep=dkeep,
+                                 gnb=None if gnb is None else (gnb, cs[4 * sum(rows[:i]) * co:]))
                 if L is None:
                     _lib.call("mvae_winograd_output_transform", m.data_ptr(), None, None, dx[b0:b1].data_ptr(), None, nb,
                               h, wd, c, mt, st)
@@ -954,11 +1015,15 @@
 
 
 def conv2d_wgrad_raw(dy, x, dw, beta: float, g: ConvGeom, db=None, x_split: bool = False, dys=None, dyb=None,
-                     x_bf16: bool = False, wino_v=None, wino_d=None, lazy=None, plan: Optional[ConvPlan] = None):
+                     x_bf16: bool = False, wino_v=None, wino_d=None, lazy=None, plan: Optional[ConvPlan] = None,
+                     dy_deferred: bool = False):
     n, c, h, wd = x.shape
     _, co, ho, wo = dy.shape
     p = plan if plan is not None else plan_conv(g, n, c, h, wd, co, _MATH[0])
     fam = _wgrad_family(p, x, dy, dw, db, x_split, dys, dyb, lazy)
+    if dy_deferred and (fam != "wino" or dys is not None or
+                        set(_kept(wino_d, p.tile, dy)) != set(tuple(ch) for ch in p.chunks)):
+        raise RuntimeError("conv2d wgrad: a deferred GroupNorm input gradient reached a kernel that reads dy")
     if lazy is not None and fam != "wino":
         x, lazy = lazy.materialize(), None
         fam = _wgrad_family(p, x, dy, dw, db, x_split, dys, dyb, None)
@@ -1093,7 +1158,7 @@
 
 class DyPack:
     __slots__ = ("bias_ref", "packed", "dx_ref", "dx_version", "dx_shape", "bias_done", "db", "fmt", "nodx",
-                 "copy_ok")
+                 "copy_ok", "defer_ok", "deferred")
 
     def __init__(self, bias_ref, fmt: str = "packed", copy_ok: bool = False):
         self.bias_ref = bias_ref
@@ -1102,8 +1167,20 @@
         self.bias_done = False
         self.nodx = False
         self.copy_ok = copy_ok
+        self.defer_ok = False
+        self.deferred = None
+
+    def take_deferred(self, dy):
+        ph, self.deferred = self.deferred, None
+        if ph is None or not isinstance(dy, DeferredGnGrad) or dy.data_ptr() != ph.data_ptr():
+            return None
+        return getattr(ph, GNB_LAZY_ATTR, None)
 
     def take(self, dy):
+        if self.deferred is not None:
+            self.deferred = None
+            raise RuntimeError("conv2d backward: the GroupNorm deferred its input gradient to this conv (its only consumer), "
+                               "but the conv's output gradient is another tensor")
         packed, ref, ver, shp, nodx = self.packed, self.dx_ref, self.dx_version, self.dx_shape, self.nodx
         out = (packed, self.bias_done, self.db)
         self.packed = self.dx_ref = self.dx_version = self.dx_shape = self.db = None
@@ -1172,6 +1249,9 @@
         ctx.gn_link = gn_link
         ctx.dx_sum = dx_sum
         ctx.dypack = dypack
+        if dypack is not None:
+            dypack.defer_ok = bool(grad_on and plan.gnb_on_load and ctx.needs_input_grad[0] and
+                                   ctx.needs_input_grad[1] and residual is None and dx_sum is None and _al16(w))
         return y
 
     @staticmethod
@@ -1183,6 +1263,17 @@
     def _backward(ctx, dy):
         x, w = ctx.saved_tensors
         g, plan = ctx.geom, ctx.plan
+        gnb = got = None
+        if isinstance(dy, DeferredGnGrad):
+            gnb = ctx.dypack.take_deferred(dy) if ctx.dypack is not None else None
+            if gnb is None:
+                raise RuntimeError("conv2d backward: a deferred GroupNorm input gradient that is not this conv's")
+            if (WINOGRAD_GNBWD_LOAD and WINOGRAD_DY2 and plan.gnb_on_load and _wgrad_wino_on(plan) and _al16(w) and
+                    ctx.needs_input_grad[0] and ctx.needs_input_grad[1] and not ctx.has_res and ctx.dx_sum is None):
+                dy = gnb.dy
+            else:
+                dy, dbm = gnb.materialize()
+                gnb, got = None, (True, True, dbm)
         dy = nhwc(dy)
         dx = dw_ret = db_ret = dres = None
         link = ctx.gn_link
@@ -1191,7 +1282,8 @@
         want_b = ctx.has_bias and ctx.needs_input_grad[2]
         bias_done = False
         dyb = None
-        got = ctx.dypack.take(dy) if ctx.dypack is not None else None
+        if got is None and gnb is None and ctx.dypack is not None:
+            got = ctx.dypack.take(dy)
         dys = None
         if got is not None:
             taken, bias_done, db_ret = got
@@ -1206,7 +1298,7 @@
                 if bt is not None:
                     bt.add_(db_ret)
                     db_ret = None
-        elif ctx.needs_input_grad[0] or ctx.needs_input_grad[1]:
+        elif gnb is None and (ctx.needs_input_grad[0] or ctx.needs_input_grad[1]):
             bt = _main_grad(ctx.bias_ref) if want_b else None
             if want_b and bt is None:
                 db_ret = torch.empty(dy.shape[1], device=dy.device, dtype=torch.float32)
@@ -1214,7 +1306,7 @@
                                      plan)
             if not bias_done:
                 db_ret = None
-        if dys is None and not g.pointwise and not _subpixel_upsample(g) and dyb is None:
+        if dys is None and not g.pointwise and not _subpixel_upsample(g) and dyb is None and gnb is None:
             dys = split_dy(dy)
         dkeep = None
 
@@ -1226,10 +1318,10 @@
             btgt = _main_grad(ctx.bias_ref) if tgt is not None and want_b and not bias_done else None
             fused = conv2d_wgrad_raw(dy, x, dw_ret if tgt is None else tgt, 0.0 if tgt is None else 1.0, g, btgt,
                                      x_split=ctx.x_split, dys=dys, dyb=dyb, x_bf16=ctx.x_bf16, wino_v=ctx.wino_v,
-                                     wino_d=dkeep, lazy=ctx.lazy, plan=plan)
+                                     wino_d=dkeep, lazy=ctx.lazy, plan=plan, dy_deferred=gnb is not None)
             bias_done = bias_done or fused
 
-        side = _bwd_side(dy) if ctx.needs_input_grad[0] and ctx.needs_input_grad[1] and \
+        side = _bwd_side(dy) if gnb is None and ctx.needs_input_grad[0] and ctx.needs_input_grad[1] and \
             _main_grad(ctx.weight_ref) is not None and not g.pointwise and min(plan.c, plan.co) >= 32 and \
             plan.ref <= BWD_OVERLAP_MAX_FLOPS else None
         if side is not None:
@@ -1256,9 +1348,19 @@
                 dx, acc.buf, acc.left = acc.buf, None, acc.n
         elif ctx.needs_input_grad[0]:
             dx = conv2d_dgrad_raw(dy, w, x.shape, g, link if ctx.x_sink is None else None, dys=dys, dyb=dyb,
-                                  dkeep=dkeep, plan=plan)
+                                  dkeep=dkeep, plan=plan, gnb=gnb)
             if ctx.x_sink is not None and ctx.x_sink.park(dx):
                 dx = None
+            if gnb is not None and want_b:
+                cs, rows = gnb.colsum
+                bt = _main_grad(ctx.bias_ref)
+                if bt is None:
+                    db_ret = torch.empty(dy.shape[1], device=dy.device, dtype=torch.float32)
+                wsb = ARENA.get("bias", _lib.query("mvae_group_norm_bwd_dy_bias_workspace_bytes", dy.shape[1]), dy.device)
+                _lib.call("mvae_group_norm_bwd_dy_bias", cs.data_ptr(), rows, dy.shape[1],
+                          (bt if bt is not None else db_ret).data_ptr(), 1.0 if bt is not None else 0.0, wsb.data_ptr(),
+                          wsb.numel(), _stream(dy))
+                bias_done = True
         if side is not None:
             main.wait_event(ev_join)
         elif ctx.needs_input_grad[1]:
@@ -1353,7 +1455,8 @@
                 y_split: bool = False, grad_sink=None, part=None, link=None, dypack=None, lazy=None,
                 conv_dy_only: bool = False):
         _check(x, "group_norm input")
-        x = nhwc(x)
+        x_in, x = x, nhwc(x)
+        ctx.x_is_input, ctx.ran_bwd = x is x_in, False
         n, c, h, w = x.shape
         mean = torch.empty(n * groups, device=x.device, dtype=torch.float32)
         rstd = torch.empty_like(mean)
@@ -1435,6 +1538,26 @@
             csb = _lib.query("mvae_group_norm_colsum_workspace_bytes", n, h * w, c)
             cs = ARENA.get("gncs", csb, x.device) if tgt is not None else None
         nodx = bool(ctx.conv_dy_only and DX_COPY_ONLY and req is not None and not bias_only and req.copy_ok)
+        if req is not None:
+            req.deferred = None
+        if (WINOGRAD_GNBWD_LOAD and gpart is not None and bias_only and req is not None and req.defer_ok and
+                ctx.conv_dy_only and add is None and ctx.x_is_input and not ctx.ran_bwd and not x.retains_grad and
+                not x._backward_hooks and _engine_runs(x.grad_fn)):
+            ctx.ran_bwd = True
+            coef = torch.empty(5 * n * c, device=x.device, dtype=torch.float32)
+            with _timed("gn_bwd", 0.0, (n, c, h * w)):
+                _lib.call("mvae_group_norm_bwd_part_coef_nhwc", gpart.data_ptr(), gamma.data_ptr(), beta.data_ptr(),
+                          mean.data_ptr(), rstd.data_ptr(), _ptr(dg), _ptr(db), n, h * w, c, groups, ws.data_ptr(),
+                          ws.numel(), coef.data_ptr(), _stream(x))
+            ph = torch.full((1,), float("nan"), device=x.device).expand(n, c, h, w).as_subclass(DeferredGnGrad)
+            setattr(ph, GNB_LAZY_ATTR, LazyGnGrad(x, dy, coef, silu, gpart, gamma, beta, mean, rstd, groups))
+            req.deferred = ph
+            if ctx.needs_input_grad[1] and dg_ret is None:
+                _grad_done(ctx.gamma_ref)
+            if ctx.needs_input_grad[2] and db_ret is None:
+                _grad_done(ctx.beta_ref)
+            return ph, dg_ret, db_ret, None, None, None, None, None, None, None, None, None, None, None, None
+        ctx.ran_bwd = True
         dxp = None if nodx else dx.data_ptr()
         if nodx and DX_POISON:
             dx.fill_(float("nan"))
```

Result: faster. 799.6 images/s, median of 6 (+1.1%).
